# GAIR-Lab/IISAN

Hardware: AMD Instinct MI355X
Metric: items/s (fwd+bwd) ViT-B+BERT-B IISAN uncached, Scientific, bs=128 (higher is better)
Workload: dtype fp16; 1 GPU; Code_Uncached IISAN ViT-base+BERT-base, Amazon-Scientific-shaped synthetic batch, bs=128/GPU (1408 item slots, all encoded), 1xMI355X per rank; global_batch=128, parallelism=dp1, encoder_blocks=all tokens in every block

## Files before the change

### iisan_amd/csrc/common.h

```cpp
#pragma once

#include <hip/hip_runtime.h>
#include <stdint.h>
#include <stdio.h>
#include <string.h>

#include "../../include/iisan_hip.h"

typedef _Float16 h8 __attribute__((ext_vector_type(8)));
typedef _Float16 h4 __attribute__((ext_vector_type(4)));
typedef __bf16 b8 __attribute__((ext_vector_type(8)));
typedef __bf16 b4 __attribute__((ext_vector_type(4)));
typedef float f4 __attribute__((ext_vector_type(4)));
typedef unsigned int u4 __attribute__((ext_vector_type(4)));
typedef unsigned int u2 __attribute__((ext_vector_type(2)));

#define WAVE 64

void iisan_set_error(const char* fmt, ...);

#define IISAN_CHECK_SHAPE(cond, ...)                                                                             \
    do {                                                                                                         \
        if (!(cond)) {                                                                                           \
            iisan_set_error(__VA_ARGS__);                                                                        \
            return IISAN_EBADSHAPE;                                                                              \
        }                                                                                                        \
    } while (0)

#define IISAN_HIP_OK(expr)                                                                                       \
    do {                                                                                                         \
        hipError_t _e = (expr);                                                                                  \
        if (_e != hipSuccess) {                                                                                  \
            iisan_set_error("%s failed at %s:%d: %s", #expr, __FILE__, __LINE__, hipGetErrorString(_e));         \
            return IISAN_EHIP;                                                                                   \
        }                                                                                                        \
    } while (0)

#define IISAN_LAUNCH_OK() IISAN_HIP_OK(hipGetLastError())

struct IisanDevKnob {
    const char* name;
    int64_t def;
    int64_t (*get)();
    void (*set)(int64_t);
};
int iisan_dev_register(const IisanDevKnob& k);
#define IISAN_DEV_KNOB(NAME, VAR)                                                                                \
    static const int iisan_dev_reg_##NAME = iisan_dev_register(IisanDevKnob{                                     \
        #NAME, (int64_t)(VAR), [] { return (int64_t)(VAR); }, [](int64_t v) { VAR = (decltype(VAR))v; }})
#define IISAN_DEV_COUNTER(NAME, VAR)                                                                             \
    static const int iisan_dev_cnt_##NAME = iisan_dev_register(IisanDevKnob{                                     \
        "count:" #NAME, INT64_MIN, [] { return (int64_t)(VAR); }, [](int64_t v) { VAR = (decltype(VAR))v; }})
#define IISAN_DEV_KNOB_FN(NAME, VAR, SET)                                                                        \
    static const int iisan_dev_reg_##NAME = iisan_dev_register(IisanDevKnob{                                     \
        #NAME, (int64_t)(VAR), [] { return (int64_t)(VAR); }, [](int64_t v) { SET; }})

#define IISAN_TRY(expr)                                                                                          \
    do {                                                                                                         \
        int _r = (expr);                                                                                         \
        if (_r != IISAN_OK) return _r;                                                                           \
    } while (0)

constexpr int IISAN_MAX_DEVICES = 64;
int iisan_cu_count();
struct OncePerDevice {
    bool done[IISAN_MAX_DEVICES] = {};
    bool first() {
        int dev = 0;
        if (hipGetDevice(&dev) != hipSuccess || dev < 0 || dev >= IISAN_MAX_DEVICES) return true;
        if (done[dev]) return false;
        done[dev] = true;
        return true;
    }
};

static inline size_t align_up(size_t x, size_t a) { return (x + a - 1) / a * a; }
static inline int64_t ceil_div(int64_t a, int64_t b) { return (a + b - 1) / b; }

struct WsCarver {
    char* base;
    size_t cap, off;
    bool overflow;
    WsCarver(void* p, size_t n) : base((char*)p), cap(n), off(0), overflow(false) {}
    template <typename T>
    T* take(size_t count) {
        size_t bytes = align_up(count * sizeof(T), 256);
        if (base && off + bytes > cap) overflow = true;
        T* r = base ? (T*)(base + off) : nullptr;
        off += bytes;
        return r;
    }
};

struct F16 {
    typedef _Float16 elem;
    typedef h8 v8;
    typedef h4 v4;
    static __device__ __forceinline__ f4 mfma(v8 a, v8 b, f4 c) {
        return __builtin_amdgcn_mfma_f32_16x16x32_f16(a, b, c, 0, 0, 0);
    }
    static __device__ __forceinline__ elem from_f32(float x) { return (_Float16)x; }
    static __device__ __forceinline__ float to_f32(elem x) { return (float)x; }
};
struct BF16 {
    typedef __bf16 elem;
    typedef b8 v8;
    typedef b4 v4;
    static __device__ __forceinline__ f4 mfma(v8 a, v8 b, f4 c) {
        return __builtin_amdgcn_mfma_f32_16x16x32_bf16(a, b, c, 0, 0, 0);
    }
    static __device__ __forceinline__ elem from_f32(float x) { return (__bf16)x; }
    static __device__ __forceinline__ float to_f32(elem x) { return (float)x; }
};

__device__ __forceinline__ float wave_sum(float v) {
#pragma unroll
    for (int o = 32; o > 0; o >>= 1) v += __shfl_xor(v, o, 64);
    return v;
}
__device__ __forceinline__ float wave_max(float v) {
#pragma unroll
    for (int o = 32; o > 0; o >>= 1) v = fmaxf(v, __shfl_xor(v, o, 64));
    return v;
}
__device__ __forceinline__ float gelu_erf(float x) { return 0.5f * x * (1.0f + erff(x * 0.70710678118654752440f)); }
constexpr float GELU_X0 = 5.5f;
__device__ __forceinline__ float gelu_absmin(float x) {
    float r;
    asm("v_min_f32 %0, |%1|, %2" : "=v"(r) : "v"(x), "v"(GELU_X0));
    return r;
}
__device__ __forceinline__ float gelu_relu(float x) {
    float r;
    asm("v_max_f32 %0, 0, %1" : "=v"(r) : "v"(x));
    return r;
}
constexpr float GELU_C0 = 9.170038104e-01f, GELU_C1 = -9.149338305e-02f, GELU_C2 = -3.171720356e-02f, GELU_C3 = -1.111552469e-03f,
                GELU_C4 = 1.940784161e-03f, GELU_C5 = -1.910830324e-04f;
__device__ __forceinline__ float gelu_erf_fast(float x) {
    const float a = gelu_absmin(x);
    float p = fmaf(a, GELU_C5, GELU_C4);
    p = fmaf(p, a, GELU_C3);
    p = fmaf(p, a, GELU_C2);
    p = fmaf(p, a, GELU_C1);
    p = fmaf(p, a, GELU_C0);
    p = p * p; p = p * p; p = p * p;
    return fmaf(-a, p, gelu_relu(x));
}
typedef float f2 __attribute__((ext_vector_type(2)));
template <int NP>
__device__ __forceinline__ void gelu_erf_fast2xN(f2* x) {
    f2 a[NP], p[NP];
#pragma unroll
    for (int k = 0; k < NP; ++k) { a[k][0] = gelu_absmin(x[k][0]); a[k][1] = gelu_absmin(x[k][1]); }
#pragma unroll
    for (int k = 0; k < NP; ++k) p[k] = __builtin_elementwise_fma(a[k], (f2)GELU_C5, (f2)GELU_C4);
#pragma unroll
    for (int k = 0; k < NP; ++k) p[k] = __builtin_elementwise_fma(p[k], a[k], (f2)GELU_C3);
#pragma unroll
    for (int k = 0; k < NP; ++k) p[k] = __builtin_elementwise_fma(p[k], a[k], (f2)GELU_C2);
#pragma unroll
    for (int k = 0; k < NP; ++k) p[k] = __builtin_elementwise_fma(p[k], a[k], (f2)GELU_C1);
#pragma unroll
    for (int k = 0; k < NP; ++k) p[k] = __builtin_elementwise_fma(p[k], a[k], (f2)GELU_C0);
#pragma unroll
    for (int sq = 0; sq < 3; ++sq)
#pragma unroll
        for (int k = 0; k < NP; ++k) p[k] = p[k] * p[k];
#pragma unroll
    for (int k = 0; k < NP; ++k) {
        f2 mx;
        mx[0] = gelu_relu(x[k][0]); mx[1] = gelu_relu(x[k][1]);
        x[k] = __builtin_elementwise_fma(-a[k], p[k], mx);
    }
}
__device__ __forceinline__ void gelu_erf_fast2x8(f2 (&x)[8]) { gelu_erf_fast2xN<8>(x); }
__device__ __forceinline__ float gelu_erf_grad(float x) {
    const float cdf = 0.5f * (1.0f + erff(x * 0.70710678118654752440f));
    const float pdf = 0.39894228040143267794f * __expf(-0.5f * x * x);
    return cdf + x * pdf;
}

__device__ __forceinline__ float drop_scale(uint64_t seed, uint32_t site, uint64_t idx, uint32_t thr24, float inv_keep) {
    uint64_t x = seed + (uint64_t)site * 0x9E3779B97F4A7C15ull + idx * 0xD1B54A32D192ED03ull;
    x ^= x >> 32; x *= 0xD6E8FEB86659FD93ull;
    x ^= x >> 32; x *= 0xD6E8FEB86659FD93ull;
    x ^= x >> 32;
    return ((uint32_t)(x >> 8) & 0xFFFFFFu) >= thr24 ? inv_keep : 0.f;
}
struct DropCfg {
    uint64_t seed;
    uint32_t site, thr24;
    float inv_keep;
};
static inline DropCfg make_drop(uint64_t seed, uint32_t site, float p) {
    DropCfg d;
    d.seed = seed; d.site = site;
    d.thr24 = p > 0.f ? (uint32_t)(p * 16777216.0f) : 0u;
    d.inv_keep = p > 0.f ? 1.0f / (1.0f - p) : 1.0f;
    return d;
}
struct RowKeepNone { static constexpr bool on = false; };
struct RowKeep {
    static constexpr bool on = true;
    DropCfg d;
    int64_t r0;
    int32_t rs;
    __device__ __forceinline__ uint64_t index(int64_t row, int D, int col) const { return (uint64_t)(r0 + row * rs) * (uint64_t)D + (uint64_t)col; }
    __device__ __forceinline__ float operator()(uint64_t idx) const { return drop_scale(d.seed, d.site, idx, d.thr24, d.inv_keep); }
};

__device__ __forceinline__ void glds16(const void* gsrc, void* lds_wave_base) {
    __builtin_amdgcn_global_load_lds((const __attribute__((address_space(1))) void*)gsrc,
                                     (__attribute__((address_space(3))) void*)lds_wave_base, 16, 0, 0);
}

__device__ __forceinline__ int xcd_remap(int bid, int nwg) {
    const int q = nwg >> 3, r = nwg & 7;
    const int xcd = bid & 7, idx = bid >> 3;
    return (xcd < r ? xcd * (q + 1) : r * (q + 1) + (xcd - r) * q) + idx;
}

bool iisan_timing_on(hipStream_t s);
int iisan_timing_class();
void iisan_timing_pre(hipStream_t s, double flops, double bytes);
void iisan_timing_post(hipStream_t s);
inline thread_local int iisan_timing_depth = 0;
struct TimedLaunch {
    hipStream_t s; int cls; bool on;
    TimedLaunch(int cls_, hipStream_t s_, double flops, double bytes)
        : s(s_), cls(cls_), on(cls_ == 1 ? iisan_timing_on(s_) : iisan_timing_class() == 2 && iisan_timing_depth == 0) {
        if (cls == 2) ++iisan_timing_depth;
        if (on) iisan_timing_pre(s, flops, bytes);
    }
    ~TimedLaunch() {
        if (cls == 2) --iisan_timing_depth;
        if (on) iisan_timing_post(s);
    }
};

struct Gemm16Args {
    const void* A;
    const void* W;
    const float* bias;
    void* out;
    const float* resid;
    const float* pos;
    int64_t M;
    int32_t N, K;
    int32_t lda, ldw, ldo;
    int32_t patch_P;
    int32_t qkv_S, qkv_heads;
    int32_t qkv_which0;
    int32_t debug;
    int32_t walk_c, walk_h;
    const float* rowstat;
    float* rowpart;
    const float* inv_a; const float* inv_b;
    int32_t atomic;
    int16_t a_blk32, out_blk32;
    int64_t split_stride;
    const int32_t* skip_last_third;
};
__host__ __device__ static inline int64_t blk32_byte(int64_t m, int64_t c, int64_t C) {
    return ((m >> 5) * (C >> 5) + (c >> 5)) * 2048 + ((c >> 3) & 1) * 1024 + (((c >> 4) & 1) * 32 + (m & 31)) * 16 + (c & 7) * 2;
}
enum { EPI_OUT16 = 0, EPI_GELU16 = 1, EPI_RESID32 = 2, EPI_PATCH32 = 3, EPI_QKVH16 = 4, EPI_F32 = 5, EPI_PATCH16 = 6, EPI_STREAM16 = 7 };
int launch_gemm16(int dtype16, int mode, const Gemm16Args& a, hipStream_t s);
enum { G16_REJECTED = -1, G16_V1 = 0, G16_S256 = 1, G16_H256 = 2 };
int gemm16_route(int dtype16, int mode, const Gemm16Args& a);
bool gemm16_s256_applicable(int mode, const Gemm16Args& a);
int launch_gemm16_s256(int dtype16, int mode, const Gemm16Args& a, hipStream_t s);
bool gemm16_h256_applicable(int mode, const Gemm16Args& a);
int launch_gemm16_h256(int dtype16, int mode, const Gemm16Args& a, hipStream_t s);
int launch_gemm16_f32(const Gemm16Args& a, int ksplit, hipStream_t s);
int launch_layernorm768(int dtype16, const float* x, const float* g, const float* b, float eps, void* out16,
                        float* out32, int64_t rows, int width, hipStream_t s);
int launch_add_layernorm768(int dtype16, const float* x, const void* delta16, const float* g, const float* b, float eps,
                            float* sum32, void* out16, float* out32, int64_t rows, int width, hipStream_t s, const RowKeep* keep = nullptr);
int launch_add2_layernorm768(int dtype16, const float* x, const void* delta16, const void* delta16b, const float* g,
                             const float* b, float eps, float* sum32, void* out16, float* out32, int64_t rows, int width, hipStream_t s,
                             const RowKeep* keep = nullptr);
enum { MX_D1 = 1, MX_D2 = 2, MX_LN = 4, MX_RESV = 8, MX_RESY = 16, MX_SRC32 = 32, MX_CLSONLY = 64, MX_POSROW = 128, MX_STAT = 256, MX_ALIAS = 512, MX_BLK32 = 1024 };
int launch_layernorm768_mixed(int dtype16, int V, const float* x32, void* x16, float* xc, const void* delta16, const void* delta16b,
                              const float* g, const float* b, float eps, void* out16, int64_t items, int Ttok, int width, hipStream_t s,
                              float* stat = nullptr, const RowKeep* keep = nullptr);
struct LnFoldJob { const void* W; const float* bias; const float* g; const float* b; void* Wf; float* bf; int32_t N;
                   int32_t w32;
};
int launch_fold_ln_weights(const LnFoldJob* jobs, int n, hipStream_t s);
int launch_stream_stats_finalize(const float* rowpart, int nslots, int64_t Mpad, void* x16, float* xc, float* rstat, float eps,
                                 int64_t items, int Ttok, hipStream_t s, bool x16_blk32 = false);
int launch_attention16(int dtype16, const void* qkv, const float* key_bias, void* ctx, int64_t items, int S,
                       int heads, hipStream_t s);
bool attention16_dma_routed(const float* key_bias, int S);
int launch_attention16_dma(int dtype16, const void* qkv, void* ctx, int64_t items, int S, int heads, hipStream_t s);
int launch_attention_cls16(int dtype16, const void* qkv, const float* key_bias, void* ctx_cls, int64_t items, int S,
                           int heads, hipStream_t s, const void* q_cls = nullptr);
int launch_vit_im2col(int dtype16, const void* img, int img_u8, void* out, int64_t M, int C, int R, int p, hipStream_t s);
int launch_vit_im2col_indexed(int dtype16, const uint8_t* catalogue, int64_t rows, const int64_t* index, void* out, int64_t M, int C,
                              int R, int p, hipStream_t s);
int launch_vit_cls_rows(float* X, const float* cls, const float* pos, int64_t M, int T, int D, hipStream_t s);
int launch_bert_embed_ln(int dtype16, const int64_t* text, const float* word, const float* pos, const float* type0,
                         const float* g, const float* b, float eps, float* X, void* H, float* key_bias, int64_t M,
                         int W, int vocab, int width, hipStream_t s, void* X16 = nullptr, float* Xc = nullptr, const RowKeep* keep = nullptr);
int launch_bert_embed_ln_indexed(int dtype16, const int64_t* table, int64_t rows, const int64_t* index, const float* word, const float* pos,
                                 const float* type0, const float* g, const float* b, float eps, float* X, void* H, float* key_bias,
                                 int64_t M, int W, int vocab, int width, hipStream_t s, void* X16 = nullptr, float* Xc = nullptr,
                                 const RowKeep* keep = nullptr);
int launch_attention16_drop(int dtype16, const void* qkv, const float* key_bias, void* ctx, int64_t items, int S, int heads,
                            const DropCfg& drop, int64_t slot0, bool cls_only, const void* q_cls, hipStream_t s);
void iisan_count_bert_drop();
int launch_gather_cls(const float* X, float* taps, int64_t M, int T, int D, int n_taps, int k, hipStream_t s);
int launch_gather_rows16(const void* H, void* out, int64_t M, int T, int D, hipStream_t s);

struct Gemm32Prob;
size_t gemm_x3_ws_bytes(int64_t M, int64_t N, int64_t K);
bool gemm_x3_applicable(const Gemm32Prob& p, int flags);
int launch_gemm_x3(const Gemm32Prob& p, int flags, void* ws, size_t ws_bytes, hipStream_t s);
size_t gemm_x3_group_ws_bytes(const int64_t* M, const int64_t* N, const int64_t* K, int n);
int launch_gemm_x3_group(const Gemm32Prob* probs, int n, int flags, void* ws, size_t ws_bytes, hipStream_t s);
int gemm_x3_group_max();
double gemm_x3_get_min_flops();
void gemm_x3_set_min_flops(double f);

struct X3pArgs {
    const _Float16* A2; const _Float16* B2;
    int64_t M; int32_t N, kp;
    const float* bias; const float* resid; float* out; int32_t ldo;
    const float* inv_a; const float* inv_b;
    const int32_t* lo_a; const int32_t* lo_b;
    int64_t split_stride;
};
int launch_gemm16_x3p(const X3pArgs& a, int ksplit, hipStream_t s);
int x3p_tile_n(int64_t M, int64_t N);

struct AmaxBatch { const float* x[16]; int64_t rows[16], cols[16], ld[16]; uint32_t* out[16]; };
int launch_amax_batch(const AmaxBatch& b, int n, hipStream_t s);

struct FuseOperands {
    const float* a; const float* b; const float* prev;
    int64_t lda, ldb, ldp;
    const float* gate;
    int32_t D, type;
};
struct Gemm32Prob {
    const float* A; const float* B; const float* bias; const float* resid; const float* act_src; float* C;
    int64_t M; int32_t N; int64_t K;
    int32_t lda, ldb, ldc, ldr;
    DropCfg drop;
    int64_t ksplit_stride;
    uint32_t* amax_a; uint32_t* amax_b;
    int32_t amax_a_ready, amax_b_ready;
    int32_t exact16_a, exact16_b;
    uint32_t* x3_zeroed;
    float* colsum_a;
};
struct N64FDesc {
    FuseOperands f;
    float* F;
    const float* W; int32_t ldw;
    const float* bias;
    float* U; float* A;
    int64_t M; int32_t K;
};
bool gemm32_n64f_ok(const N64FDesc* d, int n);
int launch_gemm32_n64f(const N64FDesc* d, int n, int gelu, hipStream_t s);
struct K64Gate { const float* gate; const float* ga; const float* go; int64_t ldga, ldgo; float* dgate; int32_t scale_prev, store; float* d2; int64_t ldd2; int32_t d2_is_b; };
bool gemm32_k64_gate_ok(const Gemm32Prob* probs, const K64Gate* gates, int nprob);
int launch_gemm32_k64_gate(const Gemm32Prob* probs, const K64Gate* gates, int nprob, hipStream_t s);
void gemm32_set_scratch(float* ws, size_t floats);
enum {
    G32_TA = 1,
    G32_TB = 2,
    G32_RELU = 4,
    G32_GELU = 8,
    G32_ACCUM = 16,
    G32_MUL_RELU_MASK = 32,
    G32_MUL_GELU_GRAD = 64,
    G32_PREACT = 128,
    G32_HINT_B_EXACT16 = 1024,
    G32_DROPOUT = 256,
};
int launch_gemm32(const Gemm32Prob* probs, int nprob, int flags, hipStream_t s);
int launch_colsum(const float* const* X, float* const* out, const int64_t* M, const int32_t* N, const int32_t* ld,
                  int nprob, hipStream_t s);

struct SanbTowerDesc {
    FuseOperands f;
    const float* Wd; const float* bd; const float* Wu; const float* bu;
    float* F; float* U; float* A; float* O;
    const float* dO; const float* Upre; float* dU; float* dprev; float* da; float* db; float* dgate; float* dbu; float* dbd;
};
bool sanb_fused_ok(int D, int down);
int launch_sanb_fwd(const SanbTowerDesc* towers, int n, int64_t M, int gelu, hipStream_t s);
int launch_sanb_bwd(const SanbTowerDesc* towers, int n, int64_t M, int gelu, hipStream_t s);
int launch_sanb_transpose(const float* const* in, float* const* out, const int32_t* rows, const int32_t* cols, int n, hipStream_t s);

struct SasFusedPtrs {
    float* Z0; float* X0;
    float* Q[8]; float* K[8]; float* V[8]; float* P[8]; float* C[8]; float* Zattn[8]; float* X1[8]; float* Hf[8]; float* Zffn[8]; float* X2[8];
};
bool sasrec_fused_ok(const iisan_sasrec_cfg* cfg);
bool sasrec_fused_shape_ok(const iisan_sasrec_cfg* cfg);
int launch_sasrec_fused_fwd(const iisan_sasrec_cfg* cfg, const float* x, const float* log_mask, int64_t B, const void* const* params,
                            float* y, const SasFusedPtrs& w, hipStream_t s);
int64_t sasrec_fused_slab_floats(const iisan_sasrec_cfg* cfg, int64_t B);
int launch_sasrec_fused_bwd(const iisan_sasrec_cfg* cfg, const float* log_mask, int64_t B, const void* const* params, const float* dy,
                            float* dx, void* const* grads, const SasFusedPtrs& w, float* slab, hipStream_t s);
```

### iisan_amd/csrc/gemm32.hip

```cpp
#include "common.h"

namespace {

constexpr int TN = 64, TK = 64, LD = 66;
__host__ __device__ constexpr int ldt(int rows) { return rows == 16 ? 48 : rows + 16; }
__host__ __device__ constexpr int smem_floats(int rows) { return rows * LD > TK * ldt(rows) ? rows * LD : TK * ldt(rows); }
typedef float f2v __attribute__((ext_vector_type(2)));

constexpr int G32_MAXP = 6;
struct Gemm32Batch {
    Gemm32Prob p[G32_MAXP];
};

template <int ROWS>
__device__ __forceinline__ void load_tile(f4 (&v)[ROWS / 16], const float* __restrict__ src, int ld, bool trans, int64_t row0,
                                          int64_t rows, int64_t k0, int64_t kend, int tid) {
    constexpr int TPR = ROWS / 4;
#pragma unroll
    for (int i = 0; i < ROWS / 16; ++i) {
        v[i] = (f4){0.f, 0.f, 0.f, 0.f};
        if (!trans) {
            const int64_t row = row0 + (tid >> 4) + 16 * i, k = k0 + (tid & 15) * 4;
            if (row < rows && k < kend) {
                const float* p = src + row * ld + k;
                if (k + 3 < kend && (((uintptr_t)p) & 15) == 0) {
                    v[i] = *(const f4*)p;
                } else {
#pragma unroll
                    for (int e = 0; e < 4; ++e)
                        if (k + e < kend) v[i][e] = p[e];
                }
            }
        } else {
            const int64_t k = k0 + tid / TPR + (256 / TPR) * i, row = row0 + (tid % TPR) * 4;
            if (k < kend && row < rows) {
                const float* p = src + k * ld + row;
                if (row + 3 < rows && (((uintptr_t)p) & 15) == 0) {
                    v[i] = *(const f4*)p;
                } else {
#pragma unroll
                    for (int e = 0; e < 4; ++e)
                        if (row + e < rows) v[i][e] = p[e];
                }
            }
        }
    }
}
template <int ROWS>
__device__ __forceinline__ void store_tile(float* S, const f4 (&v)[ROWS / 16], bool trans, int tid) {
    constexpr int TPR = ROWS / 4;
#pragma unroll
    for (int i = 0; i < ROWS / 16; ++i) {
        if (!trans) {
            float* d = S + ((tid >> 4) + 16 * i) * LD + (tid & 15) * 4;
            *(f2v*)d = (f2v){v[i][0], v[i][1]};
            *(f2v*)(d + 2) = (f2v){v[i][2], v[i][3]};
        } else {
            *(f4*)(S + (tid / TPR + (256 / TPR) * i) * ldt(ROWS) + (tid % TPR) * 4) = v[i];
        }
    }
}

template <int FLAGS, int TMV, bool FAST, int DEPTHV = 2>
__global__ __launch_bounds__(256) void gemm32_kernel(Gemm32Batch batch, int epi) {
    constexpr int TM = TMV;
    constexpr int WM = TMV >= 32 ? 2 : 1, WN = 4 / WM, FM = TMV / 16 / WM, FN = 4 / WN;
    __shared__ __attribute__((aligned(16))) float As_[smem_floats(TM)];
    __shared__ __attribute__((aligned(16))) float Bs_[smem_floats(TN)];
    float (*As)[LD] = (float (*)[LD])As_;
    const Gemm32Prob& p = batch.p[blockIdx.z];
    const int tiles_n = (p.N + TN - 1) / TN;
    const int64_t tiles_m = (p.M + TM - 1) / TM;
    if ((int64_t)blockIdx.x >= tiles_m * tiles_n) return;
    const int64_t tile_m = blockIdx.x / tiles_n;
    const int tile_n = blockIdx.x - tile_m * tiles_n;
    const int64_t m0 = tile_m * TM;
    const int n0 = tile_n * TN;

    const int64_t ktiles = (p.K + TK - 1) / TK;
    const int64_t per = (ktiles + gridDim.y - 1) / gridDim.y;
    const int64_t kbeg = (int64_t)blockIdx.y * per * TK;
    int64_t kend = kbeg + per * TK;
    if (kend > p.K) kend = p.K;
    if (kbeg >= kend && blockIdx.y > 0) return;

    const int tid = threadIdx.x, lane = tid & 63, wave = tid >> 6;
    const int wm = wave / WN, wn = wave % WN;
    const int fi = lane & 15, fk = lane >> 4;
    constexpr bool TA = (FLAGS & G32_TA) != 0, TB = (FLAGS & G32_TB) != 0;

    constexpr int KA = (FM * FN >= 4) ? 1 : 4 / (FM * FN);
    f4 acc[KA][FM][FN];
#pragma unroll
    for (int q = 0; q < KA; ++q)
#pragma unroll
        for (int a = 0; a < FM; ++a)
#pragma unroll
            for (int b = 0; b < FN; ++b) acc[q][a][b] = (f4){0.f, 0.f, 0.f, 0.f};

    constexpr int DEPTH = DEPTHV;
    f4 ra[DEPTH][TM / 16], rb[DEPTH][4];
    constexpr int TPRA = TM / 4, TPRB = TN / 4;
    const float* pa = TA ? p.A + (kbeg + tid / TPRA) * p.lda + m0 + (tid % TPRA) * 4 : p.A + (m0 + (tid >> 4)) * p.lda + kbeg + (tid & 15) * 4;
    const float* pb = TB ? p.B + (kbeg + tid / TPRB) * p.ldb + n0 + (tid % TPRB) * 4 : p.B + (int64_t)(n0 + (tid >> 4)) * p.ldb + kbeg + (tid & 15) * 4;
    const int64_t sia = TA ? (int64_t)(256 / TPRA) * p.lda : (int64_t)16 * p.lda, sib = TB ? (int64_t)(256 / TPRB) * p.ldb : (int64_t)16 * p.ldb;
    const int64_t ska = TA ? (int64_t)TK * p.lda : TK, skb = TB ? (int64_t)TK * p.ldb : TK;
    const int64_t last_t = (kend - kbeg - 1) / TK;
    auto fetch = [&](int slot, int64_t k) {
        if constexpr (FAST) {
            int64_t t = (k - kbeg) / TK;
            t = t < last_t ? t : last_t;
#pragma unroll
            for (int i = 0; i < TM / 16; ++i) ra[slot][i] = *(const f4*)(pa + t * ska + i * sia);
#pragma unroll
            for (int i = 0; i < 4; ++i) rb[slot][i] = *(const f4*)(pb + t * skb + i * sib);
            return;
        }
        if (k < kend) {
            if constexpr (FAST) {
            } else {
                load_tile<TM>(ra[slot], p.A, p.lda, TA, m0, p.M, k, kend, tid);
                load_tile<TN>(rb[slot], p.B, p.ldb, TB, n0, p.N, k, kend, tid);
            }
        }
    };
    constexpr int NP = TM / 16 + 4;
    const float* const pa_u = TA ? p.A + kbeg * p.lda + m0 : p.A + m0 * p.lda + kbeg;
    const float* const pb_u = TB ? p.B + kbeg * p.ldb + n0 : p.B + (int64_t)n0 * p.ldb + kbeg;
    uint32_t voa[TM / 16], vob[4];
#pragma unroll
    for (int i = 0; i < TM / 16; ++i)
        voa[i] = (uint32_t)(((TA ? (int64_t)(tid / TPRA) * p.lda + (tid % TPRA) * 4 : (int64_t)(tid >> 4) * p.lda + (tid & 15) * 4) + i * sia) * 4);
#pragma unroll
    for (int i = 0; i < 4; ++i)
        vob[i] = (uint32_t)(((TB ? (int64_t)(tid / TPRB) * p.ldb + (tid % TPRB) * 4 : (int64_t)(tid >> 4) * p.ldb + (tid & 15) * 4) + i * sib) * 4);
    auto fetch_piece = [&](int slot, int64_t k, int i) {
        int64_t t = (k - kbeg) / TK;
        t = t < last_t ? t : last_t;
        if (i < TM / 16) ra[slot][i] = *(const f4*)((const char*)(pa_u + t * ska) + voa[i]);
        else rb[slot][i - TM / 16] = *(const f4*)((const char*)(pb_u + t * skb) + vob[i - TM / 16]);
    };
#pragma unroll
    for (int u = 0; u < DEPTH; ++u) fetch(u, kbeg + (int64_t)u * TK);
    for (int64_t kb = kbeg; kb < kend; kb += (int64_t)DEPTH * TK) {
#pragma unroll
        for (int u = 0; u < DEPTH; ++u) {
            const int64_t k0 = kb + (int64_t)u * TK;
            if (k0 < kend) {
                store_tile<TM>(As_, ra[u], TA, tid);
                store_tile<TN>(Bs_, rb[u], TB, tid);
                __syncthreads();
                if constexpr (!FAST) fetch(u, k0 + (int64_t)DEPTH * TK);
                const int ksteps = (kend - k0 >= TK) ? TK / 4 : (int)((kend - k0 + 3) / 4);
                auto kstep = [&](int ks0) {
#pragma unroll
                    for (int q = 0; q < KA; ++q) {
                        const int ks = ks0 + q;
                        float a[FM], b[FN];
#pragma unroll
                        for (int f = 0; f < FM; ++f)
                            a[f] = TA ? As_[(ks * 4 + fk) * ldt(TM) + wm * 16 * FM + f * 16 + fi] : As_[(wm * 16 * FM + f * 16 + fi) * LD + ks * 4 + fk];
#pragma unroll
                        for (int f = 0; f < FN; ++f)
                            b[f] = TB ? Bs_[(ks * 4 + fk) * ldt(TN) + wn * 16 * FN + f * 16 + fi] : Bs_[(wn * 16 * FN + f * 16 + fi) * LD + ks * 4 + fk];
#pragma unroll
                        for (int mf = 0; mf < FM; ++mf)
#pragma unroll
                            for (int nf = 0; nf < FN; ++nf)
                                acc[q][mf][nf] = __builtin_amdgcn_mfma_f32_16x16x4f32(a[mf], b[nf], acc[q][mf][nf], 0, 0, 0);
                    }
                };
                if (FAST || ksteps == TK / 4) {
                    float ac[FM], bc[FN];
                    auto frag = [&](int ks, float (&a)[FM], float (&b)[FN]) {
#pragma unroll
                        for (int f = 0; f < FM; ++f)
                            a[f] = TA ? As_[(ks * 4 + fk) * ldt(TM) + wm * 16 * FM + f * 16 + fi] : As_[(wm * 16 * FM + f * 16 + fi) * LD + ks * 4 + fk];
#pragma unroll
                        for (int f = 0; f < FN; ++f)
                            b[f] = TB ? Bs_[(ks * 4 + fk) * ldt(TN) + wn * 16 * FN + f * 16 + fi] : Bs_[(wn * 16 * FN + f * 16 + fi) * LD + ks * 4 + fk];
                    };
                    frag(0, ac, bc);
#pragma unroll
                    for (int ks = 0; ks < TK / 4; ++ks) {
                        float an[FM], bn[FN];
                        frag(ks + 1 < TK / 4 ? ks + 1 : ks, an, bn);
                        __builtin_amdgcn_sched_barrier(0);
#pragma unroll
                        for (int mf = 0; mf < FM; ++mf)
#pragma unroll
                            for (int nf = 0; nf < FN; ++nf)
                                acc[ks % KA][mf][nf] = __builtin_amdgcn_mfma_f32_16x16x4f32(ac[mf], bc[nf], acc[ks % KA][mf][nf], 0, 0, 0);
                        if constexpr (FAST) {
                            if ((ks & 1) && (ks >> 1) < NP) fetch_piece(u, k0 + (int64_t)DEPTH * TK, ks >> 1);
                        }
                        __builtin_amdgcn_sched_barrier(0);
#pragma unroll
                        for (int f = 0; f < FM; ++f) ac[f] = an[f];
#pragma unroll
                        for (int f = 0; f < FN; ++f) bc[f] = bn[f];
                    }
                } else {
                    for (int ks0 = 0; ks0 < ksteps; ks0 += KA) kstep(ks0);
                }
                __syncthreads();
            }
        }
    }

    const bool first_split = blockIdx.y == 0;
    float* const Cp = p.C + (int64_t)blockIdx.y * p.ksplit_stride;
    constexpr bool ACC = (FLAGS & G32_ACCUM) != 0;
    const bool vec_ok = !ACC && n0 + TN <= p.N && (p.ldc & 3) == 0 && ((uintptr_t)p.C & 15) == 0 &&
                        (!p.resid || ((p.ldr & 3) == 0 && ((uintptr_t)p.resid & 15) == 0)) &&
                        (!p.act_src || ((uintptr_t)p.act_src & 15) == 0) && (!p.bias || ((uintptr_t)p.bias & 15) == 0);
    if (vec_ok) {
#pragma unroll
        for (int mf = 0; mf < FM; ++mf)
#pragma unroll
            for (int nf = 0; nf < FN; ++nf)
#pragma unroll
                for (int r = 0; r < 4; ++r) {
                    float v = acc[0][mf][nf][r];
#pragma unroll
                    for (int q = 1; q < KA; ++q) v += acc[q][mf][nf][r];
                    As[wm * 16 * FM + mf * 16 + fk * 4 + r][wn * 16 * FN + nf * 16 + fi] = v;
                }
        __syncthreads();
        for (int idx = tid; idx < TM * 16; idx += 256) {
            const int row = idx >> 4, c4 = (idx & 15) * 4;
            const int64_t m = m0 + row;
            if (m >= p.M) continue;
            const int n = n0 + c4;
            const f2v lo = *(const f2v*)&As[row][c4], hi = *(const f2v*)&As[row][c4 + 2];
            f4 v = {lo[0], lo[1], hi[0], hi[1]};
            if (p.bias && first_split) v += *(const f4*)(p.bias + n);
            const int64_t ci = m * p.ldc + n;
            if (epi & G32_PREACT) *(f4*)((float*)p.act_src + ci) = v;
            f4 act = {0.f, 0.f, 0.f, 0.f};
            if (epi & (G32_MUL_RELU_MASK | G32_MUL_GELU_GRAD)) act = *(const f4*)(p.act_src + ci);
#pragma unroll
            for (int e = 0; e < 4; ++e) {
                float x = v[e];
                if (epi & G32_RELU) x = fmaxf(x, 0.f);
                if (epi & G32_GELU) x = gelu_erf(x);
                if (epi & G32_MUL_RELU_MASK) x = act[e] > 0.f ? x : 0.f;
                if (epi & G32_MUL_GELU_GRAD) x *= gelu_erf_grad(act[e]);
                if (epi & G32_DROPOUT) x *= drop_scale(p.drop.seed, p.drop.site, (uint64_t)(ci + e), p.drop.thr24, p.drop.inv_keep);
                v[e] = x;
            }
            if (p.resid && first_split) v += *(const f4*)(p.resid + m * p.ldr + n);
            *(f4*)(Cp + ci) = v;
        }
        return;
    }
#pragma unroll
    for (int mf = 0; mf < FM; ++mf)
#pragma unroll
        for (int nf = 0; nf < FN; ++nf) {
            const int n = n0 + wn * 16 * FN + nf * 16 + fi;
            if (n >= p.N) continue;
            const float bias = (p.bias && first_split) ? p.bias[n] : 0.f;
#pragma unroll
            for (int r = 0; r < 4; ++r) {
                const int64_t m = m0 + wm * 16 * FM + mf * 16 + fk * 4 + r;
                if (m >= p.M) continue;
                float v = acc[0][mf][nf][r];
#pragma unroll
                for (int q = 1; q < KA; ++q) v += acc[q][mf][nf][r];
                v += bias;
                if (epi & G32_PREACT) ((float*)p.act_src)[m * p.ldc + n] = v;
                if (epi & G32_RELU) v = fmaxf(v, 0.f);
                if (epi & G32_GELU) v = gelu_erf(v);
                if (epi & G32_MUL_RELU_MASK) v = p.act_src[m * p.ldc + n] > 0.f ? v : 0.f;
                if (epi & G32_MUL_GELU_GRAD) v *= gelu_erf_grad(p.act_src[m * p.ldc + n]);
                if (epi & G32_DROPOUT) v *= drop_scale(p.drop.seed, p.drop.site, (uint64_t)(m * p.ldc + n), p.drop.thr24, p.drop.inv_keep);
                if (p.resid && first_split) v += p.resid[m * p.ldr + n];
                if constexpr (ACC)
                    atomicAdd(p.C + m * p.ldc + n, v);
                else
                    Cp[m * p.ldc + n] = v;
            }
        }
}

__global__ __launch_bounds__(256, 2) void gemm32_dw_kernel(Gemm32Batch batch) {
    __shared__ __attribute__((aligned(16))) float sm[2][2][64 * 64];
    const Gemm32Prob& p = batch.p[blockIdx.z];
    const int tiles_n = p.N >> 6;
    const int64_t tiles_m = p.M >> 6;
    if ((int64_t)blockIdx.x >= tiles_m * tiles_n) return;
    const int64_t tile_m = blockIdx.x / tiles_n;
    const int tile_n = (int)(blockIdx.x - tile_m * tiles_n);
    const int64_t m0 = tile_m * 64;
    const int n0 = tile_n * 64;
    const int64_t ktiles = p.K / TK;
    const int64_t per = (ktiles + gridDim.y - 1) / gridDim.y;
    const int64_t kt0 = (int64_t)blockIdx.y * per;
    int64_t kt1 = kt0 + per;
    if (kt1 > ktiles) kt1 = ktiles;
    if (kt0 >= kt1) return;
    const int tid = threadIdx.x, lane = tid & 63;
    const int wave = __builtin_amdgcn_readfirstlane(tid >> 6);
    const int i16 = lane & 15, kq = lane >> 4;
    const float* const a_u = p.A + kt0 * TK * p.lda + m0;
    const float* const b_u = p.B + kt0 * TK * p.ldb + n0;
    uint32_t voa[4], vob[4];
#pragma unroll
    for (int q = 0; q < 4; ++q) {
        voa[q] = (uint32_t)((((int64_t)(tid >> 4) + 16 * q) * p.lda + (tid & 15) * 4) * 4);
        vob[q] = (uint32_t)((((int64_t)(tid >> 4) + 16 * q) * p.ldb + (tid & 15) * 4) * 4);
    }
    const int64_t nt = kt1 - kt0;
    f4 st[2][8];
    auto piece = [&](int slot, int64_t t, int q) {
        t = t < nt ? t : nt - 1;
        if (q < 4) st[slot][q] = *(const f4*)((const char*)(a_u + t * TK * p.lda) + voa[q]);
        else st[slot][q] = *(const f4*)((const char*)(b_u + t * TK * p.ldb) + vob[q - 4]);
    };
#pragma unroll
    for (int q = 0; q < 8; ++q) piece(0, 0, q);
#pragma unroll
    for (int q = 0; q < 8; ++q) piece(1, 1, q);
    f4 acc[4][4];
#pragma unroll
    for (int e = 0; e < 4; ++e)
#pragma unroll
        for (int f = 0; f < 4; ++f) acc[e][f] = (f4){0.f, 0.f, 0.f, 0.f};
    const int sw = (tid >> 4) * 64 + (tid & 15) * 4;
    const int rd = (16 * wave + kq) * 64 + 4 * i16;
    const bool do_cs = p.colsum_a != nullptr && tile_n == 0;
    f4 csum = {0.f, 0.f, 0.f, 0.f};
    auto tile = [&](int64_t t, int slot) {
        float* bufA = sm[t & 1][0];
        float* bufB = sm[t & 1][1];
#pragma unroll
        for (int q = 0; q < 4; ++q) {
            *(f4*)(bufA + sw + 16 * 64 * q) = st[slot][q];
            *(f4*)(bufB + sw + 16 * 64 * q) = st[slot][4 + q];
            if (do_cs) csum += st[slot][q];
        }
        __builtin_amdgcn_sched_barrier(0);
        __syncthreads();
        __builtin_amdgcn_sched_barrier(0);
        f4 a = *(const f4*)(bufA + rd), b = *(const f4*)(bufB + rd);
#pragma unroll
        for (int s = 0; s < 4; ++s) {
            const f4 an = *(const f4*)(bufA + rd + 4 * 64 * (s < 3 ? s + 1 : s)), bn = *(const f4*)(bufB + rd + 4 * 64 * (s < 3 ? s + 1 : s));
            __builtin_amdgcn_sched_barrier(0);
#pragma unroll
            for (int e = 0; e < 4; ++e) {
#pragma unroll
                for (int f = 0; f < 4; ++f) acc[e][f] = __builtin_amdgcn_mfma_f32_16x16x4f32(a[e], b[f], acc[e][f], 0, 0, 0);
                if (e & 1) {
                    __builtin_amdgcn_sched_barrier(0);
                    piece(slot, t + 2, 2 * s + (e >> 1));
                    __builtin_amdgcn_sched_barrier(0);
                }
            }
            __builtin_amdgcn_sched_barrier(0);
            a = an; b = bn;
        }
    };
    int64_t t = 0;
#pragma unroll 1
    for (; t + 2 <= nt; t += 2) { tile(t, 0); tile(t + 1, 1); }
    if (t < nt) tile(t, 0);
    __syncthreads();
    float* red = &sm[0][0][0] + wave * 4096;
#pragma unroll
    for (int e = 0; e < 4; ++e)
#pragma unroll
        for (int r = 0; r < 4; ++r)
            *(f4*)(red + (16 * kq + 4 * r + e) * 64 + 4 * i16) = (f4){acc[e][0][r], acc[e][1][r], acc[e][2][r], acc[e][3][r]};
    __syncthreads();
    float* const Cp = p.C + (int64_t)blockIdx.y * p.ksplit_stride;
    const float* all = &sm[0][0][0];
#pragma unroll
    for (int q = 0; q < 4; ++q) {
        const int id = tid + 256 * q;
        const int o = (id >> 4) * 64 + (id & 15) * 4;
        const f4 v = (*(const f4*)(all + o) + *(const f4*)(all + 4096 + o)) + (*(const f4*)(all + 8192 + o) + *(const f4*)(all + 12288 + o));
        *(f4*)(Cp + (m0 + (id >> 4)) * p.ldc + n0 + (id & 15) * 4) = v;
    }
    if (do_cs) {
        __syncthreads();
        float* cs = &sm[0][0][0];
        *(f4*)(cs + (tid >> 4) * 64 + (tid & 15) * 4) = csum;
        __syncthreads();
        if (tid < 64) {
            float v = 0.f;
#pragma unroll
            for (int r = 0; r < 16; ++r) v += cs[r * 64 + tid];
            Cp[p.M * p.N + m0 + tid] = v;
        }
    }
}

struct N64FProb {
    const float* a; const float* b; const float* prev; int64_t lda, ldb, ldp; const float* gate; int32_t type;
    float* F; const float* W; int32_t ldw; const float* bias; float* U; float* A; float* P; int64_t pstride; int64_t M; int32_t K;
};
struct N64FBatch { N64FProb p[3]; int32_t gelu; int32_t rpw; };

__global__ __launch_bounds__(256, 2) void gemm32_n64f_kernel(N64FBatch batch) {
    __shared__ __attribute__((aligned(16))) float wl[2][64 * 68];
    const N64FProb& p = batch.p[blockIdx.z];
    const int64_t m0 = (int64_t)blockIdx.x * batch.rpw;
    if (m0 >= p.M) return;
    const int ktiles = p.K >> 6;
    const int per = (ktiles + (int)gridDim.y - 1) / (int)gridDim.y;
    const int kt0 = (int)blockIdx.y * per;
    int kt1 = kt0 + per;
    if (kt1 > ktiles) kt1 = ktiles;
    if (kt0 >= kt1) return;
    const int nt = kt1 - kt0;
    const int tid = threadIdx.x, lane = tid & 63;
    const int wave = __builtin_amdgcn_readfirstlane(tid >> 6);
    const int j = lane & 15, g = lane >> 4;
    const int64_t mj = m0 + 16 * wave + j;
    const int64_t mrow = mj < p.M ? mj : p.M - 1;
    const bool live = mj < p.M && 16 * wave + j < batch.rpw;
    const bool wave_on = 16 * wave < batch.rpw;
    const bool gated = p.gate != nullptr;
    const float gv = gated ? 1.0f / (1.0f + __expf(-p.gate[0] / 0.1f)) : 1.0f;
    const float ca = gated ? gv : 1.f, cb = gated ? 1.f - gv : 1.f;
    const bool has_b = p.type == 1;
    const float cp = p.prev ? (p.type == 0 ? cb : 1.f) : 0.f;
    const float* arow = p.a + mrow * p.lda + 4 * g;
    const float* prow = p.prev ? p.prev + mrow * p.ldp + 4 * g : arow;
    const float* brow = has_b ? p.b + mrow * p.ldb + 4 * g : arow;
    float* frow = p.F + mrow * (int64_t)p.K + 4 * g;
    const float* wsrc = p.W + (int64_t)(tid >> 4) * p.ldw + (tid & 15) * 4;
    const int64_t wq = (int64_t)16 * p.ldw;
    const int sw = (tid >> 4) * 68 + (tid & 15) * 4;
    f4 wst[4], an[4], pn[4], bn[4];
    auto piece = [&](int t, int q) {
        const int kk = (kt0 + (t < nt ? t : nt - 1)) * 64;
        const int s = q & 3;
        if (q < 4) an[s] = *(const f4*)(arow + kk + 16 * s);
        else if (q < 8) pn[s] = *(const f4*)(prow + kk + 16 * s);
        else if (q < 12) { if (has_b) bn[s] = *(const f4*)(brow + kk + 16 * s); }
        else wst[s] = *(const f4*)(wsrc + kk + s * wq);
    };
#pragma unroll
    for (int q = 0; q < 16; ++q) piece(0, q);
    f4 acc[4];
#pragma unroll
    for (int q = 0; q < 4; ++q) acc[q] = (f4){0.f, 0.f, 0.f, 0.f};
    const int lw = j * 68 + 4 * g;
#pragma unroll 1
    for (int t = 0; t < nt; ++t) {
        float* buf = wl[t & 1];
        const int kk = (kt0 + t) * 64;
        f4 xa[4];
#pragma unroll
        for (int s = 0; s < 4; ++s) {
            *(f4*)(buf + sw + 16 * 68 * s) = wst[s];
            f4 f = cp * pn[s] + ca * an[s];
            if (has_b) f += cb * bn[s];
            xa[s] = f;
            if (live) *(f4*)(frow + kk + 16 * s) = f;
        }
        __builtin_amdgcn_sched_barrier(0);
        __syncthreads();
        __builtin_amdgcn_sched_barrier(0);
        const float* wb = buf + lw;
        if (wave_on) {
#pragma unroll
            for (int s = 0; s < 4; ++s) {
                f4 w[4];
#pragma unroll
                for (int f = 0; f < 4; ++f) w[f] = *(const f4*)(wb + 16 * f * 68 + 16 * s);
#pragma unroll
                for (int e = 0; e < 4; ++e) {
#pragma unroll
                    for (int f = 0; f < 4; ++f) acc[f] = __builtin_amdgcn_mfma_f32_16x16x4f32(w[f][e], xa[s][e], acc[f], 0, 0, 0);
                    __builtin_amdgcn_sched_barrier(0);
                    piece(t + 1, 4 * s + e);
                    __builtin_amdgcn_sched_barrier(0);
                }
            }
        } else {
#pragma unroll
            for (int q = 12; q < 16; ++q) piece(t + 1, q);
        }
    }
    if (!live) return;
    if (gridDim.y > 1) {
        float* pr = p.P + (int64_t)blockIdx.y * p.pstride + mrow * 64 + 4 * g;
#pragma unroll
        for (int f = 0; f < 4; ++f) *(f4*)(pr + 16 * f) = acc[f];
        return;
    }
#pragma unroll
    for (int f = 0; f < 4; ++f) {
        const int n = 16 * f + 4 * g;
        f4 v = acc[f] + *(const f4*)(p.bias + n);
        *(f4*)(p.U + mrow * 64 + n) = v;
#pragma unroll
        for (int e = 0; e < 4; ++e) v[e] = batch.gelu ? gelu_erf(v[e]) : fmaxf(v[e], 0.f);
        *(f4*)(p.A + mrow * 64 + n) = v;
    }
}

struct K64Prob {
    const float* A; const float* W; const float* bias; const float* resid; float* C; int64_t M; int32_t N, lda, ldw, ldc, ldr;
    const float* gate; const float* ga; const float* go; int64_t ldga, ldgo; float* dgate; int32_t scale_prev, store;
    float* d2; int64_t ldd2; int32_t d2_is_b;
};
struct K64Batch { K64Prob p[4]; };

template <bool TBV, bool GATE = false>
__global__ __launch_bounds__(256, 2) void gemm32_k64_kernel(K64Batch batch, int nblk) {
    extern __shared__ __attribute__((aligned(16))) float wlds[];
    __shared__ float gred[4];
    const K64Prob& p = batch.p[blockIdx.z];
    const int c0 = (int)blockIdx.y * nblk * 64;
    if ((int64_t)blockIdx.x * 64 >= p.M || c0 >= p.N) return;
    int nb = (p.N - c0) >> 6;
    nb = nb < nblk ? nb : nblk;
    const int cols = nb * 64;
    const int tid = threadIdx.x, lane = tid & 63;
    const int wave = __builtin_amdgcn_readfirstlane(tid >> 6);
    const int j = lane & 15, g = lane >> 4;
    const int stride = TBV ? cols + 4 : 68;
    {
        const int per_row = TBV ? cols / 4 : 16;
        const int pieces = 16 * cols;
        f4 t[16];
#pragma unroll
        for (int q = 0; q < 16; ++q) {
            int id = tid + 256 * q;
            id = id < pieces ? id : pieces - 1;
            const int r = id / per_row, c = id - r * per_row;
            t[q] = TBV ? *(const f4*)(p.W + (int64_t)r * p.ldw + c0 + 4 * c) : *(const f4*)(p.W + (int64_t)(c0 + r) * p.ldw + 4 * c);
        }
#pragma unroll
        for (int q = 0; q < 16; ++q) {
            const int id = tid + 256 * q;
            if (id < pieces) {
                const int r = id / per_row, c = id - r * per_row;
                *(f4*)(wlds + r * stride + 4 * c) = t[q];
            }
        }
    }
    const bool has_r = p.resid != nullptr, has_b = p.bias != nullptr;
    float gpart = 0.f, gval = 0.f;
    if constexpr (GATE) gval = 1.0f / (1.0f + __expf(-p.gate[0] / 0.1f));
    const float cdp = (GATE && p.scale_prev) ? 1.f - gval : 1.f;
    const float cgo = (GATE && p.go) ? 1.f : 0.f;
    const float cd2 = GATE ? (p.d2_is_b ? 1.f - gval : gval) : 0.f;
    const float* wl = wlds + (TBV ? (16 * g) * stride + 4 * (4 * (j & 3) + (j >> 2)) : j * stride + 4 * g);
    __syncthreads();
#pragma unroll 1
    for (int64_t m0 = (int64_t)blockIdx.x * 64; m0 < p.M; m0 += (int64_t)gridDim.x * 64) {
    const int64_t mj = m0 + 16 * wave + j;
    const int64_t mrow = mj < p.M ? mj : p.M - 1;
    const bool live = mj < p.M;
    f4 xa[4];
    {
        const float* ar = p.A + mrow * p.lda + (TBV ? 16 * g : 4 * g);
#pragma unroll
        for (int q = 0; q < 4; ++q) xa[q] = *(const f4*)(ar + (TBV ? 4 * q : 16 * q));
    }
    const int ocol = c0 + 4 * g;
    float* crow = p.C + mrow * p.ldc + ocol;
    const float* rrow = has_r ? p.resid + mrow * p.ldr + ocol : crow;
    const float* brow = has_b ? p.bias + ocol : p.W + 4 * g;
    const float* garow = GATE ? p.ga + mrow * p.ldga + ocol : nullptr;
    const float* gorow = GATE ? (p.go ? p.go + mrow * p.ldgo + ocol : p.ga + mrow * p.ldga + ocol) : nullptr;
    f4 rn[4];
#pragma unroll
    for (int q = 0; q < 4; ++q) rn[q] = *(const f4*)(rrow + 16 * q);
#pragma unroll 1
    for (int t = 0; t < nb; ++t) {
        f4 wc[16];
        {
            const float* wb = wl + (TBV ? 64 * t : 64 * t * stride);
#pragma unroll
            for (int q1 = 0; q1 < (TBV ? 16 : 4); ++q1)
#pragma unroll
                for (int q2 = 0; q2 < (TBV ? 1 : 4); ++q2)
                    wc[TBV ? q1 : 4 * q1 + q2] = *(const f4*)(wb + q1 * (TBV ? stride : 16 * stride) + 16 * q2);
        }
        f4 rv[4], bv[4];
        const int tn = t + 1 < nb ? t + 1 : t;
#pragma unroll
        for (int q = 0; q < 4; ++q) {
            rv[q] = rn[q];
            bv[q] = *(const f4*)(brow + 64 * t + 16 * q);
        }
#pragma unroll
        for (int q = 0; q < 4; ++q) rn[q] = *(const f4*)(rrow + 64 * tn + 16 * q);
        f4 gav[4], gov[4];
        if constexpr (GATE) {
#pragma unroll
            for (int q = 0; q < 4; ++q) {
                gav[q] = *(const f4*)(garow + 64 * t + 16 * q);
                gov[q] = *(const f4*)(gorow + 64 * t + 16 * q);
            }
        }
        __builtin_amdgcn_sched_barrier(0);
        f4 acc[4];
#pragma unroll
        for (int q = 0; q < 4; ++q) acc[q] = (f4){0.f, 0.f, 0.f, 0.f};
        if constexpr (TBV) {
#pragma unroll
            for (int s = 0; s < 16; ++s)
#pragma unroll
                for (int e = 0; e < 4; ++e) acc[e] = __builtin_amdgcn_mfma_f32_16x16x4f32(wc[s][e], xa[s >> 2][s & 3], acc[e], 0, 0, 0);
        } else {
#pragma unroll
            for (int s = 0; s < 4; ++s)
#pragma unroll
                for (int e = 0; e < 4; ++e)
#pragma unroll
                    for (int f = 0; f < 4; ++f) acc[f] = __builtin_amdgcn_mfma_f32_16x16x4f32(wc[4 * f + s][e], xa[s][e], acc[f], 0, 0, 0);
        }
        __builtin_amdgcn_sched_barrier(0);
#pragma unroll
        for (int q = 0; q < 4; ++q) {
            const f4 v = TBV ? (f4){acc[0][q], acc[1][q], acc[2][q], acc[3][q]} : acc[q];
            const f4 z = {0.f, 0.f, 0.f, 0.f};
            const f4 o = v + ((has_b ? bv[q] : z) + (has_r ? rv[q] : z));
            if constexpr (GATE) {
                if (live) {
                    const f4 d = gav[q] - cgo * gov[q];
                    gpart += (o[0] * d[0] + o[1] * d[1]) + (o[2] * d[2] + o[3] * d[3]);
                    if (p.store) *(f4*)(crow + 64 * t + 16 * q) = o * cdp;
                    if (p.d2) *(f4*)(p.d2 + mrow * p.ldd2 + ocol + 64 * t + 16 * q) = o * cd2;
                }
            } else {
                if (live) *(f4*)(crow + 64 * t + 16 * q) = o;
            }
        }
    }
    }
    if constexpr (GATE) {
        gpart = wave_sum(gpart);
        if (lane == 0) gred[wave] = gpart;
        __syncthreads();
        if (tid == 0) atomicAdd(p.dgate, ((gred[0] + gred[1]) + (gred[2] + gred[3])) * gval * (1.f - gval) / 0.1f);
    }
}

struct ColsumBatch {
    const float* X[4];
    float* out[4];
    int64_t M[4];
    int32_t N[4], ld[4];
};
__global__ __launch_bounds__(256) void colsum_kernel(ColsumBatch b, int rows_per_block) {
    __shared__ float part[4][64];
    const int z = blockIdx.z;
    const int c = threadIdx.x & 63, rl = threadIdx.x >> 6;
    const int n = blockIdx.x * 64 + c;
    const int64_t r0 = (int64_t)blockIdx.y * rows_per_block;
    int64_t r1 = r0 + rows_per_block;
    if (r1 > b.M[z]) r1 = b.M[z];
    float s = 0.f;
    if (n < b.N[z]) {
        const float* xp = b.X[z] + n;
        const int64_t ld = b.ld[z];
        float part8[8] = {0.f, 0.f, 0.f, 0.f, 0.f, 0.f, 0.f, 0.f};
        int64_t r = r0 + rl;
        for (; r + 28 < r1; r += 32) {
#pragma unroll
            for (int u = 0; u < 8; ++u) part8[u] += xp[(r + 4 * u) * ld];
        }
        for (; r < r1; r += 4) s += xp[r * ld];
        s += ((part8[0] + part8[1]) + (part8[2] + part8[3])) + ((part8[4] + part8[5]) + (part8[6] + part8[7]));
    }
    part[rl][c] = s;
    __syncthreads();
    if (rl == 0 && n < b.N[z] && r0 < b.M[z]) atomicAdd(b.out[z] + n, part[0][c] + part[1][c] + part[2][c] + part[3][c]);
}

struct ReduceBatch { Gemm32Prob p[G32_MAXP]; const float* P[G32_MAXP]; int64_t stride[G32_MAXP]; int32_t ns[G32_MAXP]; float* cs[G32_MAXP]; };
__global__ __launch_bounds__(256) void gemm32_reduce_kernel(ReduceBatch rb, int ks_launch, int epi) {
    const Gemm32Prob& p = rb.p[blockIdx.z];
    const int ks = ks_launch < rb.ns[blockIdx.z] ? ks_launch : rb.ns[blockIdx.z];
    const float* P = rb.P[blockIdx.z];
    const int64_t stride = rb.stride[blockIdx.z], total = p.M * p.N;
    if (rb.cs[blockIdx.z]) {
        for (int64_t m = (int64_t)blockIdx.x * blockDim.x + threadIdx.x; m < p.M; m += (int64_t)gridDim.x * blockDim.x) {
            float v = 0.f;
            for (int y = 0; y < ks; ++y) v += P[(int64_t)y * stride + total + m];
            rb.cs[blockIdx.z][m] += v;
        }
    }
    if (epi == 0 && !p.bias && (p.N & 3) == 0 && (p.ldc & 3) == 0 && (!p.resid || (p.ldr & 3) == 0)) {
        const int64_t total4 = total / 4;
        const int n4 = p.N / 4;
        for (int64_t i = (int64_t)blockIdx.x * blockDim.x + threadIdx.x; i < total4; i += (int64_t)gridDim.x * blockDim.x) {
            const int64_t m = i / n4;
            const int n = (int)(i - m * n4) * 4;
            f4 acc[8];
#pragma unroll
            for (int u = 0; u < 8; ++u) acc[u] = (f4){0.f, 0.f, 0.f, 0.f};
            int y = 0;
            for (; y + 8 <= ks; y += 8) {
#pragma unroll
                for (int u = 0; u < 8; ++u) acc[u] += *(const f4*)(P + (int64_t)(y + u) * stride + 4 * i);
            }
            for (int u = 0; y < ks; ++y, ++u) acc[u] += *(const f4*)(P + (int64_t)y * stride + 4 * i);
            f4 v = ((acc[0] + acc[1]) + (acc[2] + acc[3])) + ((acc[4] + acc[5]) + (acc[6] + acc[7]));
            if (p.resid) v += *(const f4*)(p.resid + m * p.ldr + n);
            *(f4*)(p.C + m * p.ldc + n) = v;
        }
        return;
    }
    for (int64_t i = (int64_t)blockIdx.x * blockDim.x + threadIdx.x; i < total; i += (int64_t)gridDim.x * blockDim.x) {
        const int64_t m = i / p.N;
        const int n = (int)(i - m * p.N);
        float v = P[i];
        for (int y = 1; y < ks; ++y) v += P[y * stride + i];
        if (p.bias) v += p.bias[n];
        const int64_t ci = m * p.ldc + n;
        if (epi & G32_PREACT) ((float*)p.act_src)[ci] = v;
        if (epi & G32_RELU) v = fmaxf(v, 0.f);
        if (epi & G32_GELU) v = gelu_erf(v);
        if (epi & G32_MUL_RELU_MASK) v = p.act_src[ci] > 0.f ? v : 0.f;
        if (epi & G32_MUL_GELU_GRAD) v *= gelu_erf_grad(p.act_src[ci]);
        if (epi & G32_DROPOUT) v *= drop_scale(p.drop.seed, p.drop.site, (uint64_t)ci, p.drop.thr24, p.drop.inv_keep);
        if (p.resid) v += p.resid[m * p.ldr + n];
        p.C[ci] = v;
    }
}

thread_local float* g_scratch = nullptr;
thread_local size_t g_scratch_floats = 0;

template <int FLAGS, bool FAST, int DEPTH>
void launch_tiled(const Gemm32Batch& b, dim3 grid, int tm, int epi, hipStream_t s) {
    if (tm == 64) hipLaunchKernelGGL((gemm32_kernel<FLAGS, 64, FAST, DEPTH>), grid, dim3(256), 0, s, b, epi);
    else if (tm == 32) hipLaunchKernelGGL((gemm32_kernel<FLAGS, 32, FAST, DEPTH>), grid, dim3(256), 0, s, b, epi);
    else hipLaunchKernelGGL((gemm32_kernel<FLAGS, 16, FAST, DEPTH>), grid, dim3(256), 0, s, b, epi);
}
template <int FLAGS>
int launch_flags(const Gemm32Batch& b, dim3 grid, int tm, int epi, bool fast, bool deep, hipStream_t s) {
    constexpr bool DW = (FLAGS & (G32_TA | G32_TB)) == (G32_TA | G32_TB);
    if (DW && deep) launch_tiled<FLAGS, true, DW ? 3 : 2>(b, grid, tm, epi, s);
    else if (fast) launch_tiled<FLAGS, true, 2>(b, grid, tm, epi, s);
    else launch_tiled<FLAGS, false, 2>(b, grid, tm, epi, s);
    IISAN_LAUNCH_OK();
    return IISAN_OK;
}
constexpr int (*g_tiled[8])(const Gemm32Batch&, dim3, int, int, bool, bool, hipStream_t) = {
    launch_flags<0>, launch_flags<G32_TA>, launch_flags<G32_TB>, launch_flags<G32_TA | G32_TB>,
    launch_flags<G32_ACCUM>, launch_flags<G32_TA | G32_ACCUM>, launch_flags<G32_TB | G32_ACCUM>, launch_flags<G32_TA | G32_TB | G32_ACCUM>};

int nonempty_splits(int64_t ktiles, int splits) { return (int)ceil_div(ktiles, ceil_div(ktiles, (int64_t)splits)); }

int launch_reduce(ReduceBatch& rb, int n, int splitk, int epi, hipStream_t s) {
    int64_t max_mn = 0;
    for (int i = 0; i < n; ++i) {
        rb.ns[i] = nonempty_splits(ceil_div(rb.p[i].K, (int64_t)TK), splitk);
        if (rb.p[i].M * rb.p[i].N > max_mn) max_mn = rb.p[i].M * rb.p[i].N;
    }
    int64_t blocks = ceil_div(max_mn, 256);
    if (blocks > 2048) blocks = 2048;
    hipLaunchKernelGGL(gemm32_reduce_kernel, dim3((unsigned)blocks, 1, (unsigned)n), dim3(256), 0, s, rb, splitk, epi);
    IISAN_LAUNCH_OK();
    return IISAN_OK;
}

}

static int g_use_k64 = 1, g_use_dw = 1;
static int64_t g_cnt_n64f = 0, g_cnt_k64 = 0, g_cnt_dw = 0;
IISAN_DEV_COUNTER(gemm32_n64f, g_cnt_n64f);
IISAN_DEV_COUNTER(gemm32_k64, g_cnt_k64);
IISAN_DEV_COUNTER(gemm32_dw, g_cnt_dw);
IISAN_DEV_KNOB(gemm32_dw, g_use_dw);
static int g_dw_splits = 0;
IISAN_DEV_KNOB(gemm32_dw_splits, g_dw_splits);
IISAN_DEV_KNOB(gemm32_k64, g_use_k64);

void gemm32_set_scratch(float* ws, size_t floats) { g_scratch = ws; g_scratch_floats = floats; }

static int g_use_n64f = 1;
IISAN_DEV_KNOB(gemm32_n64f, g_use_n64f);
bool gemm32_n64f_ok(const N64FDesc* d, int n) {
    if (!g_use_n64f || n < 1 || n > 3) return false;
    for (int i = 0; i < n; ++i) {
        const N64FDesc& q = d[i];
        const FuseOperands& f = q.f;
        if (q.K < 256 || (q.K & 63) || (f.lda & 3) || (q.ldw & 3) || (f.prev && (f.ldp & 3)) || (f.type == 1 && (!f.b || (f.ldb & 3))) || !f.a || !q.bias ||
            (((uintptr_t)f.a | (uintptr_t)f.b | (uintptr_t)f.prev | (uintptr_t)q.F | (uintptr_t)q.W | (uintptr_t)q.bias | (uintptr_t)q.U | (uintptr_t)q.A) & 15))
            return false;
    }
    return true;
}
static void fill(N64FProb& q, const N64FDesc& d) {
    q.a = d.f.a; q.b = d.f.b; q.prev = d.f.prev; q.lda = d.f.lda; q.ldb = d.f.ldb; q.ldp = d.f.ldp; q.gate = d.f.gate; q.type = d.f.type;
    q.F = d.F; q.W = d.W; q.ldw = d.ldw; q.bias = d.bias; q.U = d.U; q.A = d.A; q.M = d.M; q.K = d.K;
}
static int launch_gemm32_n64f_impl(const N64FDesc* d, int n, int gelu, hipStream_t s) {
    IISAN_CHECK_SHAPE(gemm32_n64f_ok(d, n), "gemm32_n64f: unsupported problem");
    N64FBatch nb{};
    nb.gelu = gelu;
    int64_t maxM = 0;
    int max_k = 0;
    for (int i = 0; i < n; ++i) {
        fill(nb.p[i], d[i]);
        if (d[i].M > maxM) maxM = d[i].M;
        if (d[i].K > max_k) max_k = d[i].K;
    }
    const int cus = iisan_cu_count();
    int rpw = 64;
    if (g_use_n64f != 2 && maxM % cus == 0 && maxM / cus > 32 && maxM / cus < 64) rpw = (int)(maxM / cus);
    nb.rpw = rpw;
    const int64_t rt = ceil_div(maxM, rpw);
    IISAN_CHECK_SHAPE(rt < (1ll << 31), "gemm32: grid too large");
    int ks = 1;
    if (g_scratch && rt * n < 384) {
        ks = max_k / (4 * TK);
        if (ks > 16) ks = 16;
        while (ks >= 2) {
            int64_t need = 0;
            for (int i = 0; i < n; ++i) need += (int64_t)ks * (int64_t)align_up((size_t)(d[i].M * 64), 64);
            if ((size_t)need <= g_scratch_floats) break;
            ks >>= 1;
        }
        if (ks < 2) ks = 1;
    }
    if (ks >= 2) {
        int64_t off = 0;
        for (int i = 0; i < n; ++i) {
            nb.p[i].P = g_scratch + off;
            nb.p[i].pstride = (int64_t)align_up((size_t)(d[i].M * 64), 64);
            off += ks * nb.p[i].pstride;
        }
    }
    ++g_cnt_n64f;
    hipLaunchKernelGGL(gemm32_n64f_kernel, dim3((unsigned)rt, (unsigned)ks, (unsigned)n), dim3(256), 0, s, nb);
    IISAN_LAUNCH_OK();
    if (ks < 2) return IISAN_OK;
    ReduceBatch rb{};
    for (int i = 0; i < n; ++i) {
        Gemm32Prob& q = rb.p[i];
        q.C = d[i].A; q.ldc = 64; q.bias = d[i].bias; q.act_src = d[i].U; q.M = d[i].M; q.N = 64; q.K = d[i].K; q.ldr = 64;
        rb.P[i] = nb.p[i].P;
        rb.stride[i] = nb.p[i].pstride;
    }
    return launch_reduce(rb, n, ks, (gelu ? G32_GELU : G32_RELU) | G32_PREACT, s);
}

static bool k64_shape_ok(const Gemm32Prob& q) {
    return q.K == 64 && q.N >= 256 && (q.N & 63) == 0 && !q.act_src && q.ksplit_stride == 0 &&
           (q.lda & 3) == 0 && (q.ldb & 3) == 0 && (q.ldc & 3) == 0 && (!q.resid || (q.ldr & 3) == 0) &&
           (((uintptr_t)q.A | (uintptr_t)q.B | (uintptr_t)q.C | (uintptr_t)q.resid | (uintptr_t)q.bias) & 15) == 0;
}
struct K64Grid { int64_t rt; int nblk, ny; };
static K64Grid k64_grid(const Gemm32Prob* probs, int nprob) {
    int64_t maxM = 0;
    int maxnb = 0;
    for (int i = 0; i < nprob; ++i) {
        if (probs[i].M > maxM) maxM = probs[i].M;
        if ((probs[i].N >> 6) > maxnb) maxnb = probs[i].N >> 6;
    }
    K64Grid g;
    g.rt = ceil_div(maxM, 64);
    g.nblk = 4;
    while (g.nblk > 1 && g.rt * ceil_div(maxnb, g.nblk) * nprob < 1024) g.nblk >>= 1;
    g.ny = (int)ceil_div(maxnb, g.nblk);
    return g;
}
static void fill_k64(K64Batch& kb, const Gemm32Prob* probs, int nprob) {
    for (int i = 0; i < nprob; ++i) {
        const Gemm32Prob& q = probs[i];
        K64Prob& k = kb.p[i];
        k = K64Prob{};
        k.A = q.A; k.W = q.B; k.bias = q.bias; k.resid = q.resid; k.C = q.C; k.M = q.M; k.N = q.N;
        k.lda = q.lda; k.ldw = q.ldb; k.ldc = q.ldc; k.ldr = q.ldr;
    }
}
static int g_use_k64_gate = 1;
IISAN_DEV_KNOB(gemm32_k64_gate, g_use_k64_gate);
bool gemm32_k64_gate_ok(const Gemm32Prob* probs, const K64Gate* gates, int nprob) {
    if (!g_use_k64 || !g_use_k64_gate || nprob < 1 || nprob > 4) return false;
    for (int i = 0; i < nprob; ++i) {
        const K64Gate& g = gates[i];
        if (!k64_shape_ok(probs[i]) || !probs[i].resid || !g.gate || !g.ga || !g.dgate || (g.ldga & 3) || (g.go && (g.ldgo & 3)) || (g.d2 && ((g.ldd2 & 3) || ((uintptr_t)g.d2 & 15))) ||
            (((uintptr_t)g.ga | (uintptr_t)g.go) & 15))
            return false;
    }
    return true;
}
static int launch_gemm32_k64_gate_impl(const Gemm32Prob* probs, const K64Gate* gates, int nprob, hipStream_t s) {
    IISAN_CHECK_SHAPE(gemm32_k64_gate_ok(probs, gates, nprob), "gemm32_k64_gate: unsupported problem");
    K64Batch kb{};
    fill_k64(kb, probs, nprob);
    for (int i = 0; i < nprob; ++i) {
        K64Prob& k = kb.p[i];
        k.gate = gates[i].gate; k.ga = gates[i].ga; k.go = gates[i].go; k.ldga = gates[i].ldga; k.ldgo = gates[i].ldgo;
        k.dgate = gates[i].dgate; k.scale_prev = gates[i].scale_prev; k.store = gates[i].store;
        k.d2 = gates[i].d2; k.ldd2 = gates[i].ldd2; k.d2_is_b = gates[i].d2_is_b;
    }
    const K64Grid g = k64_grid(probs, nprob);
    IISAN_CHECK_SHAPE(g.rt < (1ll << 31), "gemm32: grid too large");
    const dim3 grid((unsigned)g.rt, (unsigned)g.ny, (unsigned)nprob);
    const size_t lds = (size_t)64 * (64 * g.nblk + 4) * sizeof(float);
    static OncePerDevice attr;
    if (attr.first())
        IISAN_HIP_OK(hipFuncSetAttribute((const void*)gemm32_k64_kernel<true, true>, hipFuncAttributeMaxDynamicSharedMemorySize, 4 * 64 * 68 * 4));
    ++g_cnt_k64;
    hipLaunchKernelGGL((gemm32_k64_kernel<true, true>), grid, dim3(256), lds, s, kb, g.nblk);
    IISAN_LAUNCH_OK();
    return IISAN_OK;
}

enum { G32K_REJECTED = -1, G32K_TILED = 0, G32K_K64 = 1, G32K_DW = 2,
       G32K_SPLIT_K64 = 3 };
enum { G32S_NONE = 0,
       G32S_EPILOGUE = 1,
       G32S_ADD_C = 2 };
enum { G32C_NONE = 0, G32C_FOLDED = 1, G32C_OWN_LAUNCH = 2 };
struct Gemm32Plan {
    int kernel;
    int tm, splitk;
    int scratch;
    bool fast, deep;
    int colsum;
    int nblk;
    int64_t gx; int gy, gz;
    int nk64;
};

static constexpr int g_tm_thresh = 512, g_splitk_target = 1024;

static int64_t partial_floats(const Gemm32Prob& q, bool with_colsum) {
    return (int64_t)align_up((size_t)(q.M * q.N + (with_colsum && q.colsum_a ? q.M : 0)), 64);
}
static bool partials_fit(const Gemm32Prob* probs, int nprob, int splitk, bool with_colsum, size_t scratch_floats) {
    int64_t need = 0;
    for (int i = 0; i < nprob; ++i) need += (int64_t)splitk * partial_floats(probs[i], with_colsum);
    return (size_t)need <= scratch_floats;
}

static Gemm32Plan plan_gemm32(const Gemm32Prob* probs, int nprob, int flags, size_t scratch_floats) {
    Gemm32Plan pl{};
    pl.kernel = G32K_REJECTED;
    if (nprob < 1 || nprob > G32_MAXP) { iisan_set_error("gemm32: 1..%d problems per launch (got %d)", G32_MAXP, nprob); return pl; }
    int64_t min_k = INT64_MAX, max_k = 0;
    bool any_colsum = false;
    for (int i = 0; i < nprob; ++i) {
        if (!(probs[i].M > 0 && probs[i].N > 0 && probs[i].K > 0)) { iisan_set_error("gemm32: empty problem %d", i); return pl; }
        if (probs[i].K < min_k) min_k = probs[i].K;
        if (probs[i].K > max_k) max_k = probs[i].K;
        any_colsum = any_colsum || probs[i].colsum_a;
    }
    const bool have_scratch = scratch_floats > 0;
    if ((flags & ~G32_TB) == 0 && g_use_k64) {
        int nk64 = 0;
        for (int i = 0; i < nprob; ++i) nk64 += k64_shape_ok(probs[i]) ? 1 : 0;
        if (nk64 > 0 && nk64 < nprob) { pl.kernel = G32K_SPLIT_K64; pl.nk64 = nk64; return pl; }
        if (nk64 == nprob && nprob <= 4) {
            const K64Grid g = k64_grid(probs, nprob);
            if (g.rt >= (1ll << 31)) { iisan_set_error("gemm32: grid too large"); return pl; }
            pl.kernel = G32K_K64; pl.nblk = g.nblk; pl.gx = g.rt; pl.gy = g.ny; pl.gz = nprob;
            return pl;
        }
    }
    auto tiles_for = [&](int tm) {
        int64_t mt = 0;
        for (int i = 0; i < nprob; ++i) {
            const int64_t t = ceil_div(probs[i].M, tm) * ceil_div(probs[i].N, TN);
            if (t > mt) mt = t;
        }
        return mt;
    };
    pl.tm = 64;
    if (!(flags & G32_ACCUM) && tiles_for(64) * nprob < g_tm_thresh) pl.tm = tiles_for(32) * nprob >= g_tm_thresh ? 32 : 16;
    const int64_t max_tiles = tiles_for(pl.tm);
    if (max_tiles >= (1ll << 31)) { iisan_set_error("gemm32: grid too large"); return pl; }
    pl.gx = max_tiles; pl.gz = nprob;
    bool dw_ok = g_use_dw && flags == (G32_TA | G32_TB | G32_ACCUM) && have_scratch;
    for (int i = 0; i < nprob && dw_ok; ++i) {
        const Gemm32Prob& q = probs[i];
        dw_ok = (q.M & 63) == 0 && (q.N & 63) == 0 && (q.K & 63) == 0 && q.K >= 4 * TK && (q.lda & 3) == 0 && (q.ldb & 3) == 0 &&
                (((uintptr_t)q.A | (uintptr_t)q.B) & 15) == 0;
    }
    pl.splitk = 1;
    if (flags & G32_ACCUM) {
        int64_t want = ceil_div(g_splitk_target, max_tiles * nprob);
        if (dw_ok) {
            int64_t sum_tiles = 0;
            for (int i = 0; i < nprob; ++i) sum_tiles += (probs[i].M >> 6) * (probs[i].N >> 6);
            const int cus = iisan_cu_count();
            want = ((int64_t)cus + sum_tiles / 2) / sum_tiles;
            if (nprob > 3) want = ((int64_t)2 * cus + sum_tiles / 2) / sum_tiles;
            if (g_dw_splits > 0 && nprob > 3) want = g_dw_splits;
        }
        const int64_t maxs = ceil_div(min_k, 2 * TK);
        pl.splitk = (int)(want < 1 ? 1 : (want > maxs ? maxs : want));
        if (have_scratch && (pl.splitk >= 2 || dw_ok)) {
            pl.splitk = nonempty_splits(ceil_div(min_k, (int64_t)TK), pl.splitk);
            if (partials_fit(probs, nprob, pl.splitk, dw_ok, scratch_floats)) pl.scratch = G32S_ADD_C;
        }
    } else if (have_scratch && max_tiles <= 192) {
        int ks = (int)(max_k / (8 * TK));
        if (ks > 8) ks = 8;
        if (ks >= 2 && partials_fit(probs, nprob, ks, false, scratch_floats)) { pl.splitk = ks; pl.scratch = G32S_EPILOGUE; }
    }
    pl.gy = pl.splitk;
    if (dw_ok && pl.scratch == G32S_ADD_C) {
        pl.kernel = G32K_DW;
        pl.colsum = any_colsum ? G32C_FOLDED : G32C_NONE;
        return pl;
    }
    pl.kernel = G32K_TILED;
    pl.fast = true;
    for (int i = 0; i < nprob && pl.fast; ++i) {
        const Gemm32Prob& q = probs[i];
        pl.fast = q.M % pl.tm == 0 && q.N % TN == 0 && q.K % TK == 0 &&
                  (q.lda & 3) == 0 && (q.ldb & 3) == 0 && ((uintptr_t)q.A & 15) == 0 && ((uintptr_t)q.B & 15) == 0;
    }
    pl.deep = pl.fast && (flags & (G32_TA | G32_TB)) == (G32_TA | G32_TB) && min_k >= 4096;
    pl.colsum = (any_colsum && (flags & G32_TA)) ? G32C_OWN_LAUNCH : G32C_NONE;
    return pl;
}

static int launch_gemm32_impl(const Gemm32Prob* probs, int nprob, int flags, hipStream_t s) {
    const Gemm32Plan pl = plan_gemm32(probs, nprob, flags, g_scratch ? g_scratch_floats : 0);
    if (pl.kernel == G32K_REJECTED) return IISAN_EBADSHAPE;
    if (pl.kernel == G32K_SPLIT_K64) {
        Gemm32Prob yes[G32_MAXP], no[G32_MAXP];
        int ny = 0, nn = 0;
        for (int i = 0; i < nprob; ++i) { if (k64_shape_ok(probs[i])) yes[ny++] = probs[i]; else no[nn++] = probs[i]; }
        IISAN_TRY(launch_gemm32_impl(yes, ny, flags, s));
        return launch_gemm32_impl(no, nn, flags, s);
    }
    const dim3 grid((unsigned)pl.gx, (unsigned)pl.gy, (unsigned)pl.gz);
    if (pl.kernel == G32K_K64) {
        K64Batch kb{};
        fill_k64(kb, probs, nprob);
        const size_t lds = (size_t)64 * pl.nblk * 68 * sizeof(float);
        static OncePerDevice attr;
        if (attr.first()) {
            IISAN_HIP_OK(hipFuncSetAttribute((const void*)gemm32_k64_kernel<true>, hipFuncAttributeMaxDynamicSharedMemorySize, 4 * 64 * 68 * 4));
            IISAN_HIP_OK(hipFuncSetAttribute((const void*)gemm32_k64_kernel<false>, hipFuncAttributeMaxDynamicSharedMemorySize, 4 * 64 * 68 * 4));
        }
        ++g_cnt_k64;
        if (flags & G32_TB) hipLaunchKernelGGL(gemm32_k64_kernel<true>, grid, dim3(256), lds, s, kb, pl.nblk);
        else hipLaunchKernelGGL(gemm32_k64_kernel<false>, grid, dim3(256), lds, s, kb, pl.nblk);
        IISAN_LAUNCH_OK();
        return IISAN_OK;
    }
    Gemm32Batch b{};
    for (int i = 0; i < nprob; ++i) b.p[i] = probs[i];
    if (pl.scratch != G32S_NONE) {
        int64_t off = 0;
        for (int i = 0; i < nprob; ++i) {
            Gemm32Prob& q = b.p[i];
            q.C = g_scratch + off; q.ldc = q.N; q.bias = nullptr; q.resid = nullptr; q.act_src = nullptr;
            q.ksplit_stride = partial_floats(q, pl.kernel == G32K_DW);
            off += pl.splitk * q.ksplit_stride;
        }
    }
    const int epi = flags & ~(G32_TA | G32_TB | G32_ACCUM);
    if (pl.kernel == G32K_DW) {
        ++g_cnt_dw;
        hipLaunchKernelGGL(gemm32_dw_kernel, grid, dim3(256), 0, s, b);
        IISAN_LAUNCH_OK();
    } else {
        const int structural = flags & (G32_TA | G32_TB | (pl.scratch == G32S_NONE ? G32_ACCUM : 0));
        const int kepi = pl.scratch == G32S_NONE ? epi : 0;
        IISAN_TRY(g_tiled[(structural & 3) | (structural & G32_ACCUM ? 4 : 0)](b, grid, pl.tm, kepi, pl.fast, pl.deep, s));
    }
    if (pl.colsum == G32C_OWN_LAUNCH) {
        const float* X[G32_MAXP]; float* O[G32_MAXP]; int64_t Ms[G32_MAXP]; int32_t Ns[G32_MAXP], lds[G32_MAXP];
        int n = 0;
        for (int i = 0; i < nprob; ++i)
            if (probs[i].colsum_a) { X[n] = probs[i].A; O[n] = probs[i].colsum_a; Ms[n] = probs[i].K; Ns[n] = (int32_t)probs[i].M; lds[n] = probs[i].lda; ++n; }
        for (int i = 0; i < n; i += 4) IISAN_TRY(launch_colsum(X + i, O + i, Ms + i, Ns + i, lds + i, n - i < 4 ? n - i : 4, s));
    }
    if (pl.scratch == G32S_NONE) return IISAN_OK;
    ReduceBatch rb{};
    for (int i = 0; i < nprob; ++i) {
        rb.p[i] = probs[i];
        if (pl.scratch == G32S_ADD_C) {
            rb.p[i].resid = probs[i].C; rb.p[i].ldr = probs[i].ldc; rb.p[i].bias = nullptr;
        }
        rb.P[i] = b.p[i].C;
        rb.stride[i] = b.p[i].ksplit_stride;
        rb.cs[i] = pl.colsum == G32C_FOLDED ? probs[i].colsum_a : nullptr;
    }
    return launch_reduce(rb, nprob, pl.splitk, epi, s);
}

extern "C" int32_t iisan_gemm32_plan(const int64_t* M, const int32_t* N, const int64_t* K, int32_t nprob, int32_t flags, int64_t scratch_floats,
                                     int32_t with_colsum, int32_t* plan12) {
    static float present[4];
    Gemm32Prob p[G32_MAXP] = {};
    for (int i = 0; i < nprob && i < G32_MAXP; ++i) {
        p[i].M = M[i]; p[i].N = N[i]; p[i].K = K[i];
        p[i].lda = (int32_t)((flags & G32_TA) ? M[i] : K[i]);
        p[i].ldb = (int32_t)((flags & G32_TB) ? N[i] : K[i]);
        p[i].ldc = N[i]; p[i].ldr = N[i];
        if (flags & (G32_PREACT | G32_MUL_RELU_MASK | G32_MUL_GELU_GRAD)) p[i].act_src = present;
        if (with_colsum) p[i].colsum_a = present;
    }
    const Gemm32Plan pl = plan_gemm32(p, nprob, flags, scratch_floats > 0 ? (size_t)scratch_floats : 0);
    const int64_t v[12] = {pl.kernel, pl.tm, pl.splitk, pl.scratch, pl.fast, pl.deep, pl.colsum, pl.nblk, pl.gx, pl.gy, pl.gz, pl.nk64};
    for (int i = 0; i < 12; ++i) plan12[i] = (int32_t)v[i];
    return pl.kernel;
}

int launch_gemm32(const Gemm32Prob* probs, int nprob, int flags, hipStream_t s) {
    double fl = 0, by = 0;
    for (int i = 0; i < nprob && i < G32_MAXP; ++i) {
        fl += 2.0 * (double)probs[i].M * probs[i].N * (double)probs[i].K;
        by += 4.0 * ((double)probs[i].M * probs[i].K + (double)probs[i].N * probs[i].K + (double)probs[i].M * probs[i].N);
    }
    TimedLaunch t(2, s, fl, by);
    return launch_gemm32_impl(probs, nprob, flags, s);
}
int launch_gemm32_n64f(const N64FDesc* d, int n, int gelu, hipStream_t s) {
    double fl = 0, by = 0;
    for (int i = 0; i < n; ++i) {
        fl += 2.0 * (double)d[i].M * 64.0 * d[i].K;
        by += 4.0 * ((double)d[i].M * d[i].K * ((d[i].f.a ? 1 : 0) + (d[i].f.b ? 1 : 0) + (d[i].f.prev ? 1 : 0) + 1) + 64.0 * d[i].K + 2.0 * d[i].M * 64.0);
    }
    TimedLaunch t(2, s, fl, by);
    return launch_gemm32_n64f_impl(d, n, gelu, s);
}
int launch_gemm32_k64_gate(const Gemm32Prob* probs, const K64Gate* gates, int nprob, hipStream_t s) {
    double fl = 0, by = 0;
    for (int i = 0; i < nprob; ++i) {
        fl += 2.0 * (double)probs[i].M * probs[i].N * 64.0;
        by += 4.0 * ((double)probs[i].M * 64.0 + (double)probs[i].N * 64.0 + 4.0 * (double)probs[i].M * probs[i].N);
    }
    TimedLaunch t(2, s, fl, by);
    return launch_gemm32_k64_gate_impl(probs, gates, nprob, s);
}

int launch_colsum(const float* const* X, float* const* out, const int64_t* M, const int32_t* N, const int32_t* ld,
                  int nprob, hipStream_t s) {
    IISAN_CHECK_SHAPE(nprob >= 1 && nprob <= 4, "colsum: 1..4 problems per launch");
    ColsumBatch b{};
    int64_t maxM = 0;
    int maxN = 0;
    for (int i = 0; i < nprob; ++i) {
        b.X[i] = X[i]; b.out[i] = out[i]; b.M[i] = M[i]; b.N[i] = N[i]; b.ld[i] = ld[i];
        if (M[i] > maxM) maxM = M[i];
        if (N[i] > maxN) maxN = N[i];
    }
    const int rows_per_block = 256;
    dim3 grid((unsigned)ceil_div(maxN, 64), (unsigned)ceil_div(maxM, rows_per_block), (unsigned)nprob);
    hipLaunchKernelGGL(colsum_kernel, grid, dim3(256), 0, s, b, rows_per_block);
    IISAN_LAUNCH_OK();
    return IISAN_OK;
}

extern "C" int iisan_gemm32(const float* A, const float* B, const float* bias, float* C, int64_t M, int32_t N, int64_t K,
                            int32_t ta, int32_t tb, int32_t relu, int32_t accumulate, void* stream) {
    Gemm32Prob p{};
    p.A = A; p.B = B; p.bias = bias; p.resid = nullptr; p.act_src = nullptr; p.C = C;
    p.M = M; p.N = N; p.K = K;
    p.lda = ta ? (int32_t)M : (int32_t)K;
    p.ldb = tb ? N : (int32_t)K;
    p.ldc = N; p.ldr = N;
    int flags = (ta ? G32_TA : 0) | (tb ? G32_TB : 0) | (relu ? G32_RELU : 0) | (accumulate ? G32_ACCUM : 0);
    return launch_gemm32(&p, 1, flags, (hipStream_t)stream);
}

extern "C" int iisan_linear_fwd(const float* x, const float* w, const float* b, float* y, int64_t M, int32_t K, int32_t N,
                                void* stream) {
    Gemm32Prob p{};
    p.A = x; p.B = w; p.bias = b; p.C = y; p.M = M; p.N = N; p.K = K; p.lda = K; p.ldb = K; p.ldc = N; p.ldr = N;
    return launch_gemm32(&p, 1, 0, (hipStream_t)stream);
}

extern "C" int iisan_linear_bwd(const float* x, const float* w, const float* dy, float* dx, float* dw, float* db,
                                int64_t M, int32_t K, int32_t N, void* stream) {
    hipStream_t s = (hipStream_t)stream;
    if (dx) {
        Gemm32Prob p{};
        p.A = dy; p.B = w; p.C = dx; p.M = M; p.N = K; p.K = N; p.lda = N; p.ldb = K; p.ldc = K; p.ldr = K;
        IISAN_TRY(launch_gemm32(&p, 1, G32_TB, s));
    }
    if (dw) {
        Gemm32Prob p{};
        p.A = dy; p.B = x; p.C = dw; p.M = N; p.N = K; p.K = M; p.lda = N; p.ldb = K; p.ldc = K; p.ldr = K;
        IISAN_TRY(launch_gemm32(&p, 1, G32_TA | G32_TB | G32_ACCUM, s));
    }
    if (db) {
        const float* X[1] = {dy};
        float* O[1] = {db};
        int64_t Ms[1] = {M};
        int32_t Ns[1] = {N}, lds[1] = {N};
        IISAN_TRY(launch_colsum(X, O, Ms, Ns, lds, 1, s));
    }
    return IISAN_OK;
}
```

### iisan_amd/csrc/sanb.hip

```cpp
#include "common.h"

namespace {


constexpr int R = 16;
constexpr int RD = 64;
constexpr int UST = RD + 4;
constexpr int NT = 256;

__device__ __forceinline__ float gate_of(const float* theta) { return 1.0f / (1.0f + __expf(-theta[0] / 0.1f)); }
__device__ __forceinline__ f4 mfma16(float a, float b, f4 c) { return __builtin_amdgcn_mfma_f32_16x16x4f32(a, b, c, 0, 0, 0); }

struct SanbTower {
    const float* a; const float* b; const float* prev;
    int64_t lda, ldb, ldp;
    const float* gate;
    int32_t D, type;
    const float* Wd; const float* bd;
    const float* Wu; const float* bu;
    float* F; float* U; float* A; float* O;
    const float* dO; const float* Upre;
    float* dU; float* dprev;
    float* da; float* db;
    float* dgate; float* dbu; float* dbd;
};
struct SanbArgs {
    SanbTower t[3];
    int64_t M;
    int32_t gelu;
};

__host__ __device__ constexpr int lds_floats(int D) { return R * (D + 4) + R * UST; }

template <int D>
__device__ __forceinline__ f4 narrow_product(const float* Xs, const float* __restrict__ W, int wave, int lane) {
    constexpr int FS = D + 4, NS = D / 16, PD = 8;
    const f4* xp = (const f4*)(Xs + (lane & 15) * FS + 4 * (lane >> 4));
    const f4* wp = (const f4*)(W + (int64_t)(wave * 16 + (lane & 15)) * D + 4 * (lane >> 4));
    f4 acc0 = {0.f, 0.f, 0.f, 0.f}, acc1 = {0.f, 0.f, 0.f, 0.f};
    f4 b[PD];
#pragma unroll
    for (int p = 0; p < PD; ++p) b[p] = wp[4 * p];
    static_assert(NS % PD == 0, "K steps");
    __builtin_amdgcn_sched_barrier(0);
    for (int s0 = 0; s0 < NS; s0 += PD) {
#pragma unroll
        for (int p = 0; p < PD; ++p) {
            const f4 a = xp[4 * (s0 + p)];
            const f4 bb = b[p];
            if (s0 + p + PD < NS) b[p] = wp[4 * (s0 + p + PD)];
            __builtin_amdgcn_sched_barrier(0);
            acc0 = mfma16(a[0], bb[0], acc0);
            acc1 = mfma16(a[1], bb[1], acc1);
            acc0 = mfma16(a[2], bb[2], acc0);
            acc1 = mfma16(a[3], bb[3], acc1);
            __builtin_amdgcn_sched_barrier(0);
        }
    }
    return acc0 + acc1;
}

template <int D>
__device__ __forceinline__ void wide_product(float* Ts, const float* Xs, const float* __restrict__ W, const float* __restrict__ bias,
                                             int wave, int lane) {
    constexpr int FS = D + 4;
    const int col = lane & 15, rg = lane >> 4;
    f4 a[4];
#pragma unroll
    for (int s = 0; s < 4; ++s) a[s] = *(const f4*)(Xs + col * UST + 16 * s + 4 * rg);
    const f4* wp = (const f4*)(W + (int64_t)(wave * (D / 4) + col) * RD + 4 * rg);
    f4 b0[4], b1[4];
#pragma unroll
    for (int s = 0; s < 4; ++s) { b0[s] = wp[4 * s]; b1[s] = wp[16 * 16 + 4 * s]; }
#pragma unroll 1
    for (int n0 = wave * (D / 4); n0 < (wave + 1) * (D / 4); n0 += 32) {
        f4 nb0[4], nb1[4];
        const bool more = n0 + 32 < (wave + 1) * (D / 4);
        if (more) {
#pragma unroll
            for (int s = 0; s < 4; ++s) { nb0[s] = wp[32 * 16 + 4 * s]; nb1[s] = wp[48 * 16 + 4 * s]; }
        }
        __builtin_amdgcn_sched_barrier(0);
        f4 c0, c1;
        float* t0 = Ts + (4 * rg) * FS + n0 + col;
        const float bi0 = bias ? bias[n0 + col] : 0.f, bi1 = bias ? bias[n0 + 16 + col] : 0.f;
#pragma unroll
        for (int r = 0; r < 4; ++r) { c0[r] = t0[r * FS] + bi0; c1[r] = t0[r * FS + 16] + bi1; }
#pragma unroll
        for (int s = 0; s < 4; ++s)
#pragma unroll
            for (int e = 0; e < 4; ++e) { c0 = mfma16(a[s][e], b0[s][e], c0); c1 = mfma16(a[s][e], b1[s][e], c1); }
#pragma unroll
        for (int r = 0; r < 4; ++r) { t0[r * FS] = c0[r]; t0[r * FS + 16] = c1[r]; }
        if (more) {
#pragma unroll
            for (int s = 0; s < 4; ++s) { b0[s] = nb0[s]; b1[s] = nb1[s]; }
        }
        wp += 32 * 16;
    }
}

template <int D>
__global__ __launch_bounds__(NT, 3) void sanb_fwd_kernel(SanbArgs args) {
    extern __shared__ __attribute__((aligned(16))) float smem[];
    const SanbTower& t = args.t[blockIdx.y];
    constexpr int FS = D + 4, d4 = D / 4;
    float* Fs = smem;
    float* As = smem + R * FS;
    const int tid = threadIdx.x, lane = tid & 63, wave = tid >> 6;
    const bool gated = t.gate != nullptr;
    const float g = gated ? gate_of(t.gate) : 1.0f;
    const int64_t ntiles = (args.M + R - 1) / R;
    for (int64_t tile = blockIdx.x; tile < ntiles; tile += gridDim.x) {
    const int64_t m0 = tile * R;

    constexpr int IT = R * d4 / NT, CH = IT % 4 == 0 ? 4 : (IT % 3 == 0 ? 3 : 1);
    for (int i0 = 0; i0 < IT; i0 += CH) {
        f4 av[CH], pv[CH], bv[CH];
#pragma unroll
        for (int j = 0; j < CH; ++j) {
            const int idx = tid + (i0 + j) * NT, row = idx / d4, c = (idx - row * d4) * 4;
            const int64_t m = m0 + row;
            av[j] = pv[j] = bv[j] = (f4){0.f, 0.f, 0.f, 0.f};
            if (m < args.M) {
                av[j] = *(const f4*)(t.a + m * t.lda + c);
                if (t.prev) pv[j] = *(const f4*)(t.prev + m * t.ldp + c);
                if (t.type == 1) bv[j] = *(const f4*)(t.b + m * t.ldb + c);
            }
        }
#pragma unroll
        for (int j = 0; j < CH; ++j) {
            const int idx = tid + (i0 + j) * NT, row = idx / d4, c = (idx - row * d4) * 4;
            const int64_t m = m0 + row;
            f4 o;
#pragma unroll
            for (int e = 0; e < 4; ++e) {
                if (t.type == 0) o[e] = gated ? g * av[j][e] + (1.f - g) * pv[j][e] : av[j][e] + pv[j][e];
                else o[e] = gated ? pv[j][e] + g * av[j][e] + (1.f - g) * bv[j][e] : pv[j][e] + av[j][e] + bv[j][e];
            }
            if (m < args.M) *(f4*)(t.F + m * D + c) = o;
            f2* fp = (f2*)(Fs + row * FS + c);
            fp[0] = (f2){o[0], o[1]};
            fp[1] = (f2){o[2], o[3]};
        }
    }
    __syncthreads();

    {
        const f4 u4 = narrow_product<D>(Fs, t.Wd, wave, lane);
        const int col = wave * 16 + (lane & 15);
        const float bd = t.bd[col];
#pragma unroll
        for (int r = 0; r < 4; ++r) {
            const int row = 4 * (lane >> 4) + r;
            const int64_t m = m0 + row;
            const float u = u4[r] + bd;
            const float a = args.gelu ? gelu_erf(u) : fmaxf(u, 0.f);
            As[row * UST + col] = a;
            if (m < args.M) {
                t.U[m * RD + col] = u;
                t.A[m * RD + col] = a;
            }
        }
    }
    __syncthreads();

    wide_product<D>(Fs, As, t.Wu, t.bu, wave, lane);
    __syncthreads();

    for (int idx = tid; idx < R * d4; idx += NT) {
        const int row = idx / d4, c = (idx - row * d4) * 4;
        const int64_t m = m0 + row;
        if (m >= args.M) continue;
        const f2* fp = (const f2*)(Fs + row * FS + c);
        const f2 lo = fp[0], hi = fp[1];
        *(f4*)(t.O + m * D + c) = (f4){lo[0], lo[1], hi[0], hi[1]};
    }
    __syncthreads();
    }
}

template <int D>
__global__ __launch_bounds__(NT, 3) void sanb_bwd_kernel(SanbArgs args) {
    extern __shared__ __attribute__((aligned(16))) float smem[];
    __shared__ float red[4];
    const SanbTower& t = args.t[blockIdx.y];
    constexpr int FS = D + 4, d4 = D / 4;
    float* Gs = smem;
    float* Ds = smem + R * FS;
    const int tid = threadIdx.x, lane = tid & 63, wave = tid >> 6;
    const bool gated = t.gate != nullptr;
    const float g = gated ? gate_of(t.gate) : 1.0f;
    const int64_t ntiles = (args.M + R - 1) / R;
    float gate_part = 0.f;
    float dbu_acc[D / NT], dbd_acc = 0.f;
#pragma unroll
    for (int i = 0; i < D / NT; ++i) dbu_acc[i] = 0.f;
    for (int64_t tile = blockIdx.x; tile < ntiles; tile += gridDim.x) {
    const int64_t m0 = tile * R;

    constexpr int IT = R * d4 / NT, CH = IT % 4 == 0 ? 4 : (IT % 3 == 0 ? 3 : 1);
    {
        f4 v[IT];
#pragma unroll
        for (int j = 0; j < IT; ++j) {
            const int idx = tid + j * NT, row = idx / d4, c = (idx - row * d4) * 4;
            const int64_t m = m0 + row;
            v[j] = (f4){0.f, 0.f, 0.f, 0.f};
            if (m < args.M) v[j] = *(const f4*)(t.dO + m * D + c);
        }
#pragma unroll
        for (int j = 0; j < IT; ++j) {
            const int idx = tid + j * NT, row = idx / d4, c = (idx - row * d4) * 4;
            f2* gp = (f2*)(Gs + row * FS + c);
            gp[0] = (f2){v[j][0], v[j][1]};
            gp[1] = (f2){v[j][2], v[j][3]};
        }
    }
    __syncthreads();

    if (t.dbu) {
#pragma unroll
        for (int i = 0; i < D / NT; ++i) {
            float s = 0.f;
#pragma unroll
            for (int row = 0; row < R; ++row) s += Gs[row * FS + tid + i * NT];
            dbu_acc[i] += s;
        }
    }

    {
        const f4 da = narrow_product<D>(Gs, t.Wd, wave, lane);
        const int col = wave * 16 + (lane & 15);
#pragma unroll
        for (int r = 0; r < 4; ++r) {
            const int row = 4 * (lane >> 4) + r;
            const int64_t m = m0 + row;
            float du = 0.f;
            if (m < args.M) {
                const float u = t.Upre[m * RD + col];
                du = da[r] * (args.gelu ? gelu_erf_grad(u) : (u > 0.f ? 1.f : 0.f));
                t.dU[m * RD + col] = du;
            }
            Ds[row * UST + col] = du;
        }
    }
    __syncthreads();
    if (t.dbd && tid < RD) {
        float s = 0.f;
#pragma unroll
        for (int row = 0; row < R; ++row) s += Ds[row * UST + tid];
        dbd_acc += s;
    }

    wide_product<D>(Gs, Ds, t.Wu, nullptr, wave, lane);
    __syncthreads();

    float part = 0.f;
    const float ca = gated ? g : 1.f, cb = gated ? 1.f - g : 1.f;
    for (int i0 = 0; i0 < IT; i0 += CH) {
        f4 av[CH], ov[CH];
#pragma unroll
        for (int j = 0; j < CH; ++j) {
            const int idx = tid + (i0 + j) * NT, row = idx / d4, c = (idx - row * d4) * 4;
            const int64_t m = m0 + row;
            av[j] = ov[j] = (f4){0.f, 0.f, 0.f, 0.f};
            if (gated && m < args.M) {
                av[j] = *(const f4*)(t.a + m * t.lda + c);
                if (t.type == 1) ov[j] = *(const f4*)(t.b + m * t.ldb + c);
                else if (t.prev) ov[j] = *(const f4*)(t.prev + m * t.ldp + c);
            }
        }
#pragma unroll
        for (int j = 0; j < CH; ++j) {
            const int idx = tid + (i0 + j) * NT, row = idx / d4, c = (idx - row * d4) * 4;
            const int64_t m = m0 + row;
            if (m >= args.M) continue;
            const f2* gp = (const f2*)(Gs + row * FS + c);
            const f2 lo = gp[0], hi = gp[1];
            const f4 df = {lo[0], lo[1], hi[0], hi[1]};
#pragma unroll
            for (int e = 0; e < 4; ++e) part += df[e] * (av[j][e] - ov[j][e]);
            if (t.da) *(f4*)(t.da + m * D + c) = (f4){ca * df[0], ca * df[1], ca * df[2], ca * df[3]};
            if (t.db) *(f4*)(t.db + m * D + c) = (f4){cb * df[0], cb * df[1], cb * df[2], cb * df[3]};
            if (t.dprev) {
                const float sc = (t.type == 0 && gated) ? cb : 1.f;
                *(f4*)(t.dprev + m * D + c) = (f4){sc * df[0], sc * df[1], sc * df[2], sc * df[3]};
            }
        }
    }
    gate_part += part;
    __syncthreads();
    }
    if (t.dbu) {
#pragma unroll
        for (int i = 0; i < D / NT; ++i) unsafeAtomicAdd(t.dbu + tid + i * NT, dbu_acc[i]);
    }
    if (t.dbd && tid < RD) unsafeAtomicAdd(t.dbd + tid, dbd_acc);
    if (gated) {
        gate_part = wave_sum(gate_part);
        if (lane == 0) red[wave] = gate_part;
        __syncthreads();
        if (tid == 0) atomicAdd(t.dgate, (red[0] + red[1] + red[2] + red[3]) * g * (1.f - g) / 0.1f);
    }
}

struct TransArgs { const float* in[6]; float* out[6]; int32_t rows[6], cols[6]; };
__global__ __launch_bounds__(256) void sanb_transpose_kernel(TransArgs a) {
    __shared__ float T[32][33];
    const int z = blockIdx.z;
    const int rows = a.rows[z], cols = a.cols[z];
    const int r0 = blockIdx.y * 32, c0 = blockIdx.x * 32;
    if (r0 >= rows || c0 >= cols) return;
    const int tx = threadIdx.x & 31, ty = threadIdx.x >> 5;
    for (int j = ty; j < 32; j += 8)
        if (r0 + j < rows && c0 + tx < cols) T[j][tx] = a.in[z][(int64_t)(r0 + j) * cols + c0 + tx];
    __syncthreads();
    for (int j = ty; j < 32; j += 8)
        if (c0 + j < cols && r0 + tx < rows) a.out[z][(int64_t)(c0 + j) * rows + r0 + tx] = T[tx][j];
}

size_t lds_bytes(int D) { return (size_t)lds_floats(D) * sizeof(float); }

}

bool sanb_fused_ok(int D, int down) { return down == RD && (D == 1024 || D == 768 || D == 512 || D == 256); }

static void fill(SanbTower& t, const SanbTowerDesc& d) {
    t.a = d.f.a; t.b = d.f.b; t.prev = d.f.prev; t.lda = d.f.lda; t.ldb = d.f.ldb; t.ldp = d.f.ldp; t.gate = d.f.gate; t.D = d.f.D; t.type = d.f.type;
    t.Wd = d.Wd; t.bd = d.bd; t.Wu = d.Wu; t.bu = d.bu; t.F = d.F; t.U = d.U; t.A = d.A; t.O = d.O;
    t.dO = d.dO; t.Upre = d.Upre; t.dU = d.dU; t.dprev = d.dprev; t.da = d.da; t.db = d.db; t.dgate = d.dgate; t.dbu = d.dbu; t.dbd = d.dbd;
}

template <bool BWD>
static int launch_sanb(const SanbTowerDesc* towers, int n, int64_t M, int gelu, hipStream_t s) {
    IISAN_CHECK_SHAPE(n >= 1 && n <= 3 && M > 0, "sanb: 1..3 towers per launch");
    SanbArgs a{};
    a.M = M; a.gelu = gelu;
    const int D = towers[0].f.D;
    for (int i = 0; i < n; ++i) {
        IISAN_CHECK_SHAPE(towers[i].f.D == D && sanb_fused_ok(D, RD), "sanb: towers of one launch must share a supported width");
        fill(a.t[i], towers[i]);
    }
    const int cus = iisan_cu_count();
    const int64_t ntile = ceil_div(M, R);
    const unsigned gx = (unsigned)(ntile > cus ? cus : ntile);
    const dim3 grid(gx, (unsigned)n), block(NT);
    const size_t lds = lds_bytes(D);
#define SANB_LAUNCH(DD)                                                                                                \
    do {                                                                                                               \
        auto k = BWD ? sanb_bwd_kernel<DD> : sanb_fwd_kernel<DD>;                                                      \
        static OncePerDevice attr;                                                                                     \
        if (attr.first())                                                                                              \
            IISAN_HIP_OK(hipFuncSetAttribute((const void*)k, hipFuncAttributeMaxDynamicSharedMemorySize, (int)lds_bytes(DD))); \
        hipLaunchKernelGGL(k, grid, block, lds, s, a);                                                                 \
    } while (0)
    switch (D) {
        case 256: SANB_LAUNCH(256); break;
        case 512: SANB_LAUNCH(512); break;
        case 768: SANB_LAUNCH(768); break;
        case 1024: SANB_LAUNCH(1024); break;
        default: iisan_set_error("sanb: width %d", D); return IISAN_EBADSHAPE;
    }
#undef SANB_LAUNCH
    IISAN_LAUNCH_OK();
    return IISAN_OK;
}

static int64_t g_cnt_sanb_fwd = 0, g_cnt_sanb_bwd = 0;
IISAN_DEV_COUNTER(sanb_fused_fwd, g_cnt_sanb_fwd);
IISAN_DEV_COUNTER(sanb_fused_bwd, g_cnt_sanb_bwd);
int launch_sanb_fwd(const SanbTowerDesc* towers, int n, int64_t M, int gelu, hipStream_t s) { ++g_cnt_sanb_fwd; return launch_sanb<false>(towers, n, M, gelu, s); }
int launch_sanb_bwd(const SanbTowerDesc* towers, int n, int64_t M, int gelu, hipStream_t s) { ++g_cnt_sanb_bwd; return launch_sanb<true>(towers, n, M, gelu, s); }

int launch_sanb_transpose(const float* const* in, float* const* out, const int32_t* rows, const int32_t* cols, int n, hipStream_t s) {
    IISAN_CHECK_SHAPE(n >= 1 && n <= 6, "sanb_transpose: 1..6 matrices per launch");
    TransArgs a{};
    int mr = 0, mc = 0;
    for (int i = 0; i < n; ++i) {
        a.in[i] = in[i]; a.out[i] = out[i]; a.rows[i] = rows[i]; a.cols[i] = cols[i];
        if (rows[i] > mr) mr = rows[i];
        if (cols[i] > mc) mc = cols[i];
    }
    hipLaunchKernelGGL(sanb_transpose_kernel, dim3((unsigned)ceil_div(mc, 32), (unsigned)ceil_div(mr, 32), (unsigned)n), dim3(256), 0, s, a);
    IISAN_LAUNCH_OK();
    return IISAN_OK;
}
```

### iisan_amd/csrc/sidenet.hip

```cpp
#include "common.h"

namespace {

struct FuseTower {
    const float* a; const float* b; const float* prev;
    int64_t lda, ldb, ldp;
    const float* gate;
    float* F;
    float* da; float* db;
    float* dgate;
    int32_t D, type;
};
struct FuseArgs {
    FuseTower t[3];
    int64_t M;
};

__device__ __forceinline__ float gate_of(const float* theta) { return 1.0f / (1.0f + __expf(-theta[0] / 0.1f)); }

__global__ __launch_bounds__(256) void fuse_fwd_kernel(FuseArgs args) {
    const FuseTower& t = args.t[blockIdx.y];
    const int d4 = t.D / 4;
    const int64_t total = args.M * d4;
    const bool gated = t.gate != nullptr;
    const float g = gated ? gate_of(t.gate) : 1.0f;
    const int64_t i0 = (int64_t)blockIdx.x * blockDim.x + threadIdx.x, step = (int64_t)gridDim.x * blockDim.x;
    const int64_t dm = step / d4;
    const int dc = (int)(step - dm * d4);
    int64_t m = i0 / d4;
    int c4 = (int)(i0 - m * d4);
    for (int64_t i = i0; i < total; i += step, m += dm, c4 += dc) {
        if (c4 >= d4) { c4 -= d4; ++m; }
        const int c = c4 * 4;
        const f4 av = *(const f4*)(t.a + m * t.lda + c);
        f4 pv = {0.f, 0.f, 0.f, 0.f}, bv = {0.f, 0.f, 0.f, 0.f};
        if (t.prev) pv = *(const f4*)(t.prev + m * t.ldp + c);
        if (t.type == 1) bv = *(const f4*)(t.b + m * t.ldb + c);
        f4 o;
#pragma unroll
        for (int e = 0; e < 4; ++e) {
            if (t.type == 0) o[e] = gated ? g * av[e] + (1.f - g) * pv[e] : av[e] + pv[e];
            else o[e] = gated ? pv[e] + g * av[e] + (1.f - g) * bv[e] : pv[e] + av[e] + bv[e];
        }
        *(f4*)(t.F + m * t.D + c) = o;
    }
}

__global__ __launch_bounds__(256) void fuse_bwd_kernel(FuseArgs args) {
    __shared__ float red[4];
    const FuseTower& t = args.t[blockIdx.y];
    const int d4 = t.D / 4;
    const int64_t total = args.M * d4;
    const bool gated = t.gate != nullptr;
    const float g = gated ? gate_of(t.gate) : 1.0f;
    float part = 0.f;
    const int64_t i0 = (int64_t)blockIdx.x * blockDim.x + threadIdx.x, step = (int64_t)gridDim.x * blockDim.x;
    const int64_t dm = step / d4;
    const int dc = (int)(step - dm * d4);
    int64_t m = i0 / d4;
    int c4 = (int)(i0 - m * d4);
    constexpr int CH = 4;
    const float ca = gated ? g : 1.f, cb = gated ? 1.f - g : 1.f;
    for (int64_t i = i0; i < total; i += CH * step) {
        f4 df[CH], av[CH], ov[CH];
        int64_t mm[CH];
        int cc[CH];
#pragma unroll
        for (int j = 0; j < CH; ++j) {
            if (c4 >= d4) { c4 -= d4; ++m; }
            mm[j] = m; cc[j] = c4 * 4;
            df[j] = av[j] = ov[j] = (f4){0.f, 0.f, 0.f, 0.f};
            if (i + j * step < total) {
                df[j] = *(const f4*)(t.F + m * t.D + cc[j]);
                if (gated) {
                    av[j] = *(const f4*)(t.a + m * t.lda + cc[j]);
                    if (t.type == 1) ov[j] = *(const f4*)(t.b + m * t.ldb + cc[j]);
                    else if (t.prev) ov[j] = *(const f4*)(t.prev + m * t.ldp + cc[j]);
                }
            }
            m += dm; c4 += dc;
        }
#pragma unroll
        for (int j = 0; j < CH; ++j) {
            if (i + j * step >= total) continue;
#pragma unroll
            for (int e = 0; e < 4; ++e) part += df[j][e] * (av[j][e] - ov[j][e]);
            const int64_t o = mm[j] * t.D + cc[j];
            if (t.da) *(f4*)(t.da + o) = (f4){ca * df[j][0], ca * df[j][1], ca * df[j][2], ca * df[j][3]};
            if (t.db) *(f4*)(t.db + o) = (f4){cb * df[j][0], cb * df[j][1], cb * df[j][2], cb * df[j][3]};
            if (t.type == 0 && gated) *(f4*)(t.F + o) = (f4){cb * df[j][0], cb * df[j][1], cb * df[j][2], cb * df[j][3]};
        }
    }
    if (!gated) return;
    part = wave_sum(part);
    if ((threadIdx.x & 63) == 0) red[threadIdx.x >> 6] = part;
    __syncthreads();
    if (threadIdx.x == 0) atomicAdd(t.dgate, (red[0] + red[1] + red[2] + red[3]) * g * (1.f - g) / 0.1f);
}

struct Plan {
    int n[3];
    int D[3];
    int H[3];
    int r, E;
    int diff_cv, diff_t;
    bool align;
    bool text_wide;
    int p_adapter[3], p_gate[3], p_dp, p_fc[3], p_head[3], n_params;
    int wd(int z, int k) const { return p_adapter[z] + 4 * k; }
    int gate(int z, int k) const { return p_gate[z] + k; }
    int dpw(int i) const { return p_dp + 2 * i; }
};

int make_plan(const iisan_side_cfg* c, Plan& p) {
    IISAN_CHECK_SHAPE(c->n_side >= 1 && c->n_side <= IISAN_MAX_SIDE, "side_net: n_side %d out of range", c->n_side);
    const int n_t = c->versa ? c->n_side_text : c->n_side;
    IISAN_CHECK_SHAPE(n_t >= 1 && n_t <= IISAN_MAX_SIDE, "side_net: n_side_text %d out of range", n_t);
    IISAN_CHECK_SHAPE(c->dim_cv % 4 == 0 && c->dim_text % 4 == 0 && c->down % 4 == 0 && c->emb % 4 == 0,
                      "side_net: widths must be multiples of 4");
    IISAN_CHECK_SHAPE(c->versa || c->dim_cv == c->dim_text, "side_net: towers of different width (%d vs %d) need versa = 1 "
                      "(Code_Cached_Asym)", c->dim_cv, c->dim_text);
    p.n[0] = c->n_side; p.n[1] = n_t; p.n[2] = p.n[0] < p.n[1] ? p.n[0] : p.n[1];
    p.D[0] = c->dim_cv; p.D[1] = c->dim_text; p.D[2] = c->dim_cv < c->dim_text ? c->dim_cv : c->dim_text;
    p.r = c->down; p.E = c->emb;
    p.diff_cv = p.n[0] > p.n[1] ? p.n[0] - p.n[1] : 0;
    p.diff_t = p.n[1] > p.n[0] ? p.n[1] - p.n[0] : 0;
    p.align = c->versa && c->dim_cv != c->dim_text;
    p.text_wide = c->dim_text > c->dim_cv;
    if (c->versa) { p.H[0] = p.E; p.H[1] = p.E; p.H[2] = p.D[2]; }
    else { p.H[0] = p.D[0]; p.H[1] = p.D[1]; p.H[2] = p.D[2]; }
    int o = 0;
    for (int z = 0; z < 3; ++z) { p.p_adapter[z] = o; o += 4 * p.n[z]; }
    for (int z = 0; z < 3; ++z) { p.p_gate[z] = o; o += p.n[z]; }
    p.p_dp = o; if (p.align) o += 2 * p.n[2];
    for (int z = 0; z < 3; ++z) { p.p_fc[z] = o; o += 2; }
    for (int z = 0; z < 3; ++z) { p.p_head[z] = o; o += 2; }
    p.n_params = o;
    for (int k = 0; k < p.n[0]; ++k)
        IISAN_CHECK_SHAPE(c->tap_index[k] >= 0 && c->tap_index[k] < c->tap_stride_cv, "side_net: cv tap index %d outside the tap tensor", c->tap_index[k]);
    for (int k = 0; k < p.n[1]; ++k) {
        const int ti = c->versa ? c->tap_index_text[k] : c->tap_index[k];
        IISAN_CHECK_SHAPE(ti >= 0 && ti < c->tap_stride_text, "side_net: text tap index %d outside the tap tensor", ti);
    }
    return IISAN_OK;
}

struct SideBufs {
    float* F[IISAN_MAX_SIDE][3];
    float* U[IISAN_MAX_SIDE][3];
    float* A[IISAN_MAX_SIDE][3];
    float* O[IISAN_MAX_SIDE][3];
    float* DP[IISAN_MAX_SIDE];
    float* Y[3];
    float* dO[3];
    float* dY[3];
    float* dU[3];
    float* dDP[IISAN_MAX_SIDE];
    void* x3; size_t x3_bytes;
    float* WT[3][2];
    float* skws; size_t skws_floats;
    uint32_t* amax;
    uint32_t* x3z_f; uint32_t* zb; uint32_t* x3z_b;
    mutable uint32_t* x3z_next; mutable int x3z_left;
};
constexpr int X3Z_WORDS = 12, X3Z_SLOTS_F = IISAN_MAX_SIDE + 4, X3Z_SLOTS_B = IISAN_MAX_SIDE + 8, ZB_HEAD = 4;

int g_use_x3 = 1;
constexpr int64_t SANB_FUSED_MAX_ROWS = 4096;
int g_use_sanb = 1;
int g_dw_merge = 1;

uint64_t x3_route_word() {
    const float f = (float)gemm_x3_get_min_flops();
    uint32_t bits;
    memcpy(&bits, &f, 4);
    return ((uint64_t)(g_use_x3 ? 1 : 0) << 32) | bits;
}

size_t x3_need(const Plan& p, int64_t M) {
    if (!g_use_x3) return 0;
    size_t need = 0;
    int64_t gm[IISAN_MAX_SIDE], gn[IISAN_MAX_SIDE], gk[IISAN_MAX_SIDE];
    int ng = 0;
    auto consider = [&](int64_t m, int64_t n, int64_t k) {
        Gemm32Prob q{};
        q.M = m; q.N = (int32_t)n; q.K = k; q.lda = q.ldb = q.ldc = q.ldr = 4;
        if (gemm_x3_applicable(q, 0) && ng < IISAN_MAX_SIDE) { gm[ng] = m; gn[ng] = n; gk[ng] = k; ++ng; }
    };
    auto close_group = [&]() {
        for (int i = 0; i < ng; i += 8) {
            const size_t b = gemm_x3_group_ws_bytes(gm + i, gn + i, gk + i, ng - i < 8 ? ng - i : 8);
            if (b > need) need = b;
        }
        ng = 0;
    };
    for (int z = 0; z < 3; ++z) consider(M, p.H[z], p.D[z]);
    close_group();
    for (int z = 0; z < 3; ++z) consider(M, p.D[z], p.H[z]);
    close_group();
    for (int z = 0; z < 3; ++z) consider(p.H[z], p.D[z], M);
    close_group();
    if (p.align) {
        const int dw = p.text_wide ? p.D[1] : p.D[0];
        for (int i = 0; i < p.n[2]; ++i) consider(M, p.D[2], dw);
        close_group();
        for (int i = 0; i < p.n[2]; ++i) consider(p.D[2], dw, M);
        close_group();
    }
    return need;
}

void carve(WsCarver& c, SideBufs& b, const Plan& p, int64_t M) {
    for (int z = 0; z < 3; ++z)
        for (int k = 0; k < p.n[z]; ++k) {
            b.F[k][z] = c.take<float>((size_t)M * p.D[z]);
            b.U[k][z] = c.take<float>((size_t)M * p.r);
            b.A[k][z] = c.take<float>((size_t)M * p.r);
            b.O[k][z] = c.take<float>((size_t)M * p.D[z]);
        }
    for (int i = 0; i < p.n[2]; ++i) b.DP[i] = p.align ? c.take<float>((size_t)M * p.D[2]) : nullptr;
    for (int z = 0; z < 3; ++z) {
        b.Y[z] = c.take<float>((size_t)M * p.H[z]);
        b.dO[z] = c.take<float>((size_t)M * p.D[z]);
        b.dY[z] = c.take<float>((size_t)M * p.H[z]);
        b.dU[z] = c.take<float>((size_t)M * p.r);
    }
    for (int i = 0; i < p.n[2]; ++i) b.dDP[i] = p.align ? c.take<float>((size_t)M * p.D[2]) : nullptr;
    for (int z = 0; z < 3; ++z) {
        b.WT[z][0] = c.take<float>((size_t)p.D[z] * p.r);
        b.WT[z][1] = c.take<float>((size_t)p.D[z] * p.r);
    }
    b.skws_floats = (size_t)3 * 8 * align_up((size_t)M * p.r, 64);
    {
        size_t wg = 0;
        for (int z = 0; z < 3; ++z) wg += (size_t)2 * 32 * align_up((size_t)p.D[z] * p.r + p.D[z], 64);
        if (wg > b.skws_floats) b.skws_floats = wg;
    }
    b.skws = c.take<float>(b.skws_floats);
    {
        uint32_t* zf = c.take<uint32_t>(16 + IISAN_MAX_SIDE + X3Z_WORDS * X3Z_SLOTS_F);
        b.amax = zf; b.x3z_f = zf ? zf + 16 + IISAN_MAX_SIDE : nullptr;
        b.zb = c.take<uint32_t>(ZB_HEAD + X3Z_WORDS * X3Z_SLOTS_B);
        b.x3z_b = b.zb ? b.zb + ZB_HEAD : nullptr;
        b.x3z_next = nullptr; b.x3z_left = 0;
    }
    b.x3_bytes = x3_need(p, M);
    b.x3 = b.x3_bytes ? (void*)c.take<char>(b.x3_bytes) : nullptr;
}

int gemm_group(const Gemm32Prob* pr, int n, int flags, const SideBufs& b, hipStream_t s) {
    Gemm32Prob rest[IISAN_MAX_SIDE], big[IISAN_MAX_SIDE];
    int nr = 0, nb = 0;
    IISAN_CHECK_SHAPE(n <= IISAN_MAX_SIDE, "gemm_group: %d problems", n);
    for (int i = 0; i < n; ++i) {
        if (b.x3 && gemm_x3_applicable(pr[i], flags)) {
            Gemm32Prob q = pr[i];
            if (b.x3z_left > 0) { q.x3_zeroed = b.x3z_next; b.x3z_next += X3Z_WORDS; --b.x3z_left; }
            big[nb++] = q;
        }
        else rest[nr++] = pr[i];
    }
    if (nb > 1 || (nb == 1 && big[0].x3_zeroed)) {
        AmaxBatch ab{};
        int na = 0;
        auto want = [&](const float* x, bool trans, int64_t op_rows, int64_t K, int64_t ld, uint32_t* slot) {
            for (int k = 0; k < na; ++k) if (ab.out[k] == slot) return;
            if (na >= 16) return;
            ab.x[na] = x; ab.rows[na] = trans ? K : op_rows; ab.cols[na] = trans ? op_rows : K; ab.ld[na] = ld; ab.out[na] = slot;
            ++na;
        };
        for (int i = 0; i < nb; ++i) {
            Gemm32Prob& q = big[i];
            if (!q.x3_zeroed && !(q.amax_a && q.amax_b)) continue;
            uint32_t* pa = q.amax_a ? q.amax_a : q.x3_zeroed;
            uint32_t* pb = q.amax_b ? q.amax_b : q.x3_zeroed + 1;
            const bool full = na + 2 > 16;
            if (full) break;
            if (!q.amax_a_ready) want(q.A, (flags & G32_TA) != 0, q.M, q.K, q.lda, pa);
            if (!q.amax_b_ready) want(q.B, (flags & G32_TB) != 0, q.N, q.K, q.ldb, pb);
            q.amax_a = pa; q.amax_b = pb; q.amax_a_ready = 1; q.amax_b_ready = 1;
        }
        IISAN_TRY(launch_amax_batch(ab, na, s));
    }
    const int gmax = gemm_x3_group_max();
    for (int i = 0; i < nb; i += gmax) IISAN_TRY(launch_gemm_x3_group(big + i, nb - i < gmax ? nb - i : gmax, flags, b.x3, b.x3_bytes, s));
    if (nr > 1 && !(flags & G32_ACCUM)) {
        int64_t kmin = INT64_MAX;
        for (int i = 0; i < nr; ++i) kmin = rest[i].K < kmin ? rest[i].K : kmin;
        for (int i = 0; i < nr;) {
            if (rest[i].N <= 64 && rest[i].K >= 4096 && rest[i].K >= 4 * kmin) {
                IISAN_TRY(launch_gemm32(&rest[i], 1, flags & ~G32_HINT_B_EXACT16, s));
                for (int k = i; k + 1 < nr; ++k) rest[k] = rest[k + 1];
                --nr;
            } else ++i;
        }
    }
    for (int i = 0; i < nr; i += 4)
        IISAN_TRY(launch_gemm32(rest + i, nr - i < 4 ? nr - i : 4, flags & ~G32_HINT_B_EXACT16, s));
    return IISAN_OK;
}

Gemm32Prob prob(const float* A, int lda, const float* B, int ldb, const float* bias, float* C, int ldc, int64_t M, int N,
                int64_t K, const float* resid = nullptr, int ldr = 0, const float* act_src = nullptr) {
    Gemm32Prob p{};
    p.A = A; p.B = B; p.bias = bias; p.resid = resid; p.act_src = act_src; p.C = C;
    p.M = M; p.N = N; p.K = K; p.lda = lda; p.ldb = ldb; p.ldc = ldc; p.ldr = ldr ? ldr : ldc;
    return p;
}

unsigned ew_grid(int64_t M, int D) {
    const int64_t b = ceil_div(M * (D / 4), 256);
    return (unsigned)(b < 4096 ? b : 4096);
}

struct StepMap {
    int nact; int z[3]; int k[3]; int mm_i;
};
StepMap step_map(const Plan& p, int g) {
    StepMap s{};
    const int diff = p.diff_cv + p.diff_t;
    if (g < diff) {
        s.nact = 1; s.z[0] = p.diff_cv ? 0 : 1; s.k[0] = g; s.mm_i = -1;
    } else {
        const int i = g - diff;
        s.nact = 3; s.mm_i = i;
        s.z[0] = 0; s.k[0] = i + p.diff_cv;
        s.z[1] = 1; s.k[1] = i + p.diff_t;
        s.z[2] = 2; s.k[2] = i;
    }
    return s;
}

struct ScratchGuard {
    ScratchGuard(float* p, size_t n) { gemm32_set_scratch(p, n); }
    ~ScratchGuard() { gemm32_set_scratch(nullptr, 0); }
};

void fill(FuseTower& t, const FuseOperands& f) {
    t.a = f.a; t.b = f.b; t.prev = f.prev; t.lda = f.lda; t.ldb = f.ldb; t.ldp = f.ldp; t.gate = f.gate; t.D = f.D; t.type = f.type;
}
K64Gate k64_gate(const FuseOperands& f) {
    K64Gate g{};
    g.gate = f.gate; g.ga = f.a; g.ldga = f.lda;
    if (f.type == 1) { g.go = f.b; g.ldgo = f.ldb; }
    else { g.go = f.prev; g.ldgo = f.ldp; }
    g.scale_prev = f.type == 0 ? 1 : 0;
    return g;
}

bool step_fusable(const Plan& p, const StepMap& sm, int64_t M) {
    if (!g_use_sanb || (g_use_sanb == 1 && M >= SANB_FUSED_MAX_ROWS)) return false;
    const int D = p.D[sm.z[0]];
    for (int a = 0; a < sm.nact; ++a)
        if (p.D[sm.z[a]] != D) return false;
    return sanb_fused_ok(D, p.r);
}

struct Ctx {
    const iisan_side_cfg* cfg; Plan p; SideBufs b;
    const float* taps[2]; int64_t M;
    const void* const* params;
    void* const* grads;
    hipStream_t s;
    const float* W(int i) const { return (const float*)params[i]; }
    float* G(int i) const { return (float*)grads[i]; }
    int tap_idx(int z, int k) const { return (z == 1 && cfg->versa) ? cfg->tap_index_text[k] : cfg->tap_index[k]; }
    int64_t tap_ld(int z) const { return (int64_t)(z == 0 ? cfg->tap_stride_cv : cfg->tap_stride_text) * p.D[z]; }
    const float* tap(int z, int k) const { return taps[z] + (int64_t)tap_idx(z, k) * p.D[z]; }
    int first_idx(int z) const { return (z == 1 && cfg->versa) ? cfg->first_index_text : cfg->first_index; }
    FuseOperands fuse_operands(int z, int k, const StepMap& sm) const {
        FuseOperands t{};
        t.D = p.D[z];
        t.gate = cfg->gated ? W(p.gate(z, k)) : nullptr;
        t.prev = nullptr; t.ldp = p.D[z];
        if (k > 0) t.prev = b.O[k - 1][z];
        else if (cfg->remove_first && z != 2) { t.prev = taps[z] + (int64_t)first_idx(z) * p.D[z]; t.ldp = tap_ld(z); }
        if (z != 2) {
            t.type = 0; t.a = tap(z, k); t.lda = tap_ld(z); t.b = nullptr; t.ldb = 0;
        } else {
            t.type = 1;
            const int kc = sm.k[0], kt = sm.k[1];
            t.a = tap(0, kc); t.lda = tap_ld(0);
            t.b = tap(1, kt); t.ldb = tap_ld(1);
            if (p.align) {
                if (p.text_wide) { t.b = b.DP[k]; t.ldb = p.D[2]; }
                else { t.a = b.DP[k]; t.lda = p.D[2]; }
            }
        }
        return t;
    }
    Gemm32Prob fc_prob(int z) const { return prob(b.O[p.n[z] - 1][z], p.D[z], W(p.p_fc[z]), p.D[z], W(p.p_fc[z] + 1), b.Y[z], p.H[z], M, p.H[z], p.D[z]); }
    Gemm32Prob align_prob(int i) const {
        const int zw = p.text_wide ? 1 : 0, kw = step_map(p, p.diff_cv + p.diff_t + i).k[zw];
        return prob(tap(zw, kw), (int)tap_ld(zw), W(p.dpw(i)), p.D[zw], W(p.dpw(i) + 1), b.DP[i], p.D[2], M, p.D[2], p.D[zw]);
    }

    int fwd_dim_align(bool taps_preset) const {
        Gemm32Prob pd[IISAN_MAX_SIDE];
        for (int i = 0; i < p.n[2]; ++i) {
            pd[i] = align_prob(i);
            pd[i].amax_a = b.amax + 9 + i;
            pd[i].amax_a_ready = taps_preset ? 1 : 0;
            pd[i].exact16_a = taps_preset ? 1 : 0;
        }
        return gemm_group(pd, p.n[2], 0, b, s);
    }

    int fwd_step_fused(const StepMap& sm) const {
        SanbTowerDesc td[3];
        for (int a = 0; a < sm.nact; ++a) {
            const int z = sm.z[a], k = sm.k[a];
            td[a] = SanbTowerDesc{};
            td[a].f = fuse_operands(z, k, sm);
            td[a].Wd = W(p.wd(z, k)); td[a].bd = W(p.wd(z, k) + 1); td[a].Wu = W(p.wd(z, k) + 2); td[a].bu = W(p.wd(z, k) + 3);
            td[a].F = b.F[k][z]; td[a].U = b.U[k][z]; td[a].A = b.A[k][z]; td[a].O = b.O[k][z];
        }
        return launch_sanb_fwd(td, sm.nact, M, cfg->gelu, s);
    }

    int fwd_step_separate(const StepMap& sm) const {
        const int na = sm.nact;
        FuseOperands fo[3];
        for (int a = 0; a < na; ++a) fo[a] = fuse_operands(sm.z[a], sm.k[a], sm);
        Gemm32Prob pr[3];
        bool fed = false;
        if (p.r == 64) {
            N64FDesc nd[3];
            for (int a = 0; a < na; ++a) {
                const int z = sm.z[a], k = sm.k[a];
                nd[a] = N64FDesc{};
                nd[a].f = fo[a];
                nd[a].F = b.F[k][z]; nd[a].W = W(p.wd(z, k)); nd[a].ldw = p.D[z]; nd[a].bias = W(p.wd(z, k) + 1);
                nd[a].U = b.U[k][z]; nd[a].A = b.A[k][z]; nd[a].M = M; nd[a].K = p.D[z];
            }
            if (gemm32_n64f_ok(nd, na)) {
                IISAN_TRY(launch_gemm32_n64f(nd, na, cfg->gelu, s));
                fed = true;
            }
        }
        if (!fed) {
            FuseArgs fa{};
            fa.M = M;
            int maxD = 0;
            for (int a = 0; a < na; ++a) {
                const int z = sm.z[a], k = sm.k[a];
                fill(fa.t[a], fo[a]);
                fa.t[a].F = b.F[k][z];
                if (p.D[z] > maxD) maxD = p.D[z];
                pr[a] = prob(b.F[k][z], p.D[z], W(p.wd(z, k)), p.D[z], W(p.wd(z, k) + 1), b.A[k][z], p.r, M, p.r, p.D[z], nullptr, 0, b.U[k][z]);
            }
            hipLaunchKernelGGL(fuse_fwd_kernel, dim3(ew_grid(M, maxD), na), dim3(256), 0, s, fa);
            IISAN_LAUNCH_OK();
            IISAN_TRY(launch_gemm32(pr, na, (cfg->gelu ? G32_GELU : G32_RELU) | G32_PREACT, s));
        }
        for (int a = 0; a < na; ++a) {
            const int z = sm.z[a], k = sm.k[a];
            pr[a] = prob(b.A[k][z], p.r, W(p.wd(z, k) + 2), p.r, W(p.wd(z, k) + 3), b.O[k][z], p.D[z], M, p.D[z], p.r, b.F[k][z], p.D[z]);
        }
        return launch_gemm32(pr, na, 0, s);
    }

    int fwd_fc_head(float* item3) const {
        Gemm32Prob pr[3];
        for (int z = 0; z < 3; ++z) {
            pr[z] = fc_prob(z);
            pr[z].amax_a = b.amax + z;
            pr[z].amax_b = b.amax + 3 + z;
        }
        IISAN_TRY(gemm_group(pr, 3, 0, b, s));
        for (int z = 0; z < 3; ++z) pr[z] = prob(b.Y[z], p.H[z], W(p.p_head[z]), p.H[z], W(p.p_head[z] + 1), item3 + z * p.E, 3 * p.E, M, p.E, p.H[z]);
        return launch_gemm32(pr, 3, 0, s);
    }

    int bwd_fc_head(const float* d_item3) const {
        const int E = p.E;
        Gemm32Prob pr[3];
        const float* cs_x[3]; float* cs_o[3]; int64_t cs_m[3] = {M, M, M}; int32_t cs_n[3], cs_ld[3];
        for (int z = 0; z < 3; ++z) pr[z] = prob(d_item3 + z * E, 3 * E, W(p.p_head[z]), p.H[z], nullptr, b.dY[z], p.H[z], M, p.H[z], E);
        IISAN_TRY(launch_gemm32(pr, 3, G32_TB, s));
        for (int z = 0; z < 3; ++z) pr[z] = prob(d_item3 + z * E, 3 * E, b.Y[z], p.H[z], nullptr, G(p.p_head[z]), p.H[z], E, p.H[z], M);
        IISAN_TRY(launch_gemm32(pr, 3, G32_TA | G32_TB | G32_ACCUM, s));
        for (int z = 0; z < 3; ++z) { cs_x[z] = d_item3 + z * E; cs_o[z] = G(p.p_head[z] + 1); cs_n[z] = E; cs_ld[z] = 3 * E; }
        IISAN_TRY(launch_colsum(cs_x, cs_o, cs_m, cs_n, cs_ld, 3, s));
        IISAN_HIP_OK(hipMemsetAsync(b.zb, 0, (size_t)(ZB_HEAD + X3Z_WORDS * X3Z_SLOTS_B) * sizeof(uint32_t), s));
        b.x3z_next = b.x3z_b; b.x3z_left = X3Z_SLOTS_B;
        int fwd_x3[3];
        for (int z = 0; z < 3; ++z) fwd_x3[z] = (b.x3 && gemm_x3_applicable(fc_prob(z), 0)) ? 1 : 0;
        for (int z = 0; z < 3; ++z) {
            pr[z] = prob(b.dY[z], p.H[z], W(p.p_fc[z]), p.D[z], nullptr, b.dO[z], p.D[z], M, p.D[z], p.H[z]);
            pr[z].amax_a = b.zb + z;
            if (fwd_x3[z]) { pr[z].amax_b = b.amax + 3 + z; pr[z].amax_b_ready = 1; }
        }
        IISAN_TRY(gemm_group(pr, 3, G32_TB, b, s));
        int dy_ready[3];
        for (int z = 0; z < 3; ++z) dy_ready[z] = (b.x3 && gemm_x3_applicable(pr[z], G32_TB)) ? 1 : 0;
        for (int z = 0; z < 3; ++z) {
            pr[z] = prob(b.dY[z], p.H[z], b.O[p.n[z] - 1][z], p.D[z], nullptr, G(p.p_fc[z]), p.D[z], p.H[z], p.D[z], M);
            pr[z].amax_a = b.zb + z; pr[z].amax_a_ready = dy_ready[z];
            if (fwd_x3[z]) { pr[z].amax_b = b.amax + z; pr[z].amax_b_ready = 1; }
        }
        IISAN_TRY(gemm_group(pr, 3, G32_TA | G32_TB | G32_ACCUM, b, s));
        for (int z = 0; z < 3; ++z) { cs_x[z] = b.dY[z]; cs_o[z] = G(p.p_fc[z] + 1); cs_n[z] = p.H[z]; cs_ld[z] = p.H[z]; }
        return launch_colsum(cs_x, cs_o, cs_m, cs_n, cs_ld, 3, s);
    }

    int bwd_step_fused(const StepMap& sm) const {
        const int na = sm.nact, r = p.r;
        Gemm32Prob pr[3];
        for (int a = 0; a < na; ++a) {
            const int z = sm.z[a], k = sm.k[a];
            pr[a] = prob(b.dO[z], p.D[z], b.A[k][z], r, nullptr, G(p.wd(z, k) + 2), r, p.D[z], r, M);
        }
        IISAN_TRY(launch_gemm32(pr, na, G32_TA | G32_TB | G32_ACCUM, s));
        SanbTowerDesc td[3];
        const float* tin[6]; float* tout[6]; int32_t trows[6], tcols[6];
        for (int a = 0; a < na; ++a) {
            const int z = sm.z[a], k = sm.k[a];
            tin[2 * a] = W(p.wd(z, k)); tout[2 * a] = b.WT[z][0]; trows[2 * a] = p.r; tcols[2 * a] = p.D[z];
            tin[2 * a + 1] = W(p.wd(z, k) + 2); tout[2 * a + 1] = b.WT[z][1]; trows[2 * a + 1] = p.D[z]; tcols[2 * a + 1] = p.r;
            td[a] = SanbTowerDesc{};
            td[a].f = fuse_operands(z, k, sm);
            td[a].Wd = b.WT[z][1]; td[a].Wu = b.WT[z][0];
            td[a].dO = b.dO[z]; td[a].Upre = b.U[k][z]; td[a].dU = b.dU[z];
            td[a].dprev = k > 0 ? b.dO[z] : nullptr;
            td[a].dgate = cfg->gated ? G(p.gate(z, k)) : nullptr;
            td[a].dbu = G(p.wd(z, k) + 3); td[a].dbd = G(p.wd(z, k) + 1);
        }
        IISAN_TRY(launch_sanb_transpose(tin, tout, trows, tcols, 2 * na, s));
        IISAN_TRY(launch_sanb_bwd(td, na, M, cfg->gelu, s));
        for (int a = 0; a < na; ++a) {
            const int z = sm.z[a], k = sm.k[a];
            pr[a] = prob(b.dU[z], r, b.F[k][z], p.D[z], nullptr, G(p.wd(z, k)), p.D[z], r, p.D[z], M);
        }
        return launch_gemm32(pr, na, G32_TA | G32_TB | G32_ACCUM, s);
    }

    int bwd_step_separate(const StepMap& sm) const {
        const int na = sm.nact, r = p.r;
        Gemm32Prob pr[3];
        for (int a = 0; a < na; ++a) {
            const int z = sm.z[a], k = sm.k[a];
            pr[a] = prob(b.dO[z], p.D[z], W(p.wd(z, k) + 2), r, nullptr, b.dU[z], r, M, r, p.D[z], nullptr, 0, b.U[k][z]);
        }
        IISAN_TRY(launch_gemm32(pr, na, G32_TB | (cfg->gelu ? G32_MUL_GELU_GRAD : G32_MUL_RELU_MASK), s));
        {
            Gemm32Prob pw[6];
            for (int a = 0; a < na; ++a) {
                const int z = sm.z[a], k = sm.k[a];
                pw[a] = prob(b.dO[z], p.D[z], b.A[k][z], r, nullptr, G(p.wd(z, k) + 2), r, p.D[z], r, M);
                pw[a].colsum_a = G(p.wd(z, k) + 3);
                pw[na + a] = prob(b.dU[z], r, b.F[k][z], p.D[z], nullptr, G(p.wd(z, k)), p.D[z], r, p.D[z], M);
                pw[na + a].colsum_a = G(p.wd(z, k) + 1);
            }
            if (g_dw_merge) IISAN_TRY(launch_gemm32(pw, 2 * na, G32_TA | G32_TB | G32_ACCUM, s));
            else {
                IISAN_TRY(launch_gemm32(pw, na, G32_TA | G32_TB | G32_ACCUM, s));
                IISAN_TRY(launch_gemm32(pw + na, na, G32_TA | G32_TB | G32_ACCUM, s));
            }
        }
        const bool need_dp = sm.mm_i >= 0 && p.align;
        FuseOperands fo[3];
        for (int a = 0; a < na; ++a) {
            const int z = sm.z[a], k = sm.k[a];
            fo[a] = fuse_operands(z, k, sm);
            pr[a] = prob(b.dU[z], r, W(p.wd(z, k)), p.D[z], nullptr, b.dO[z], p.D[z], M, p.D[z], r, b.dO[z], p.D[z]);
        }
        if (cfg->gated) {
            K64Gate kg[3];
            for (int a = 0; a < na; ++a) {
                const int z = sm.z[a], k = sm.k[a];
                kg[a] = k64_gate(fo[a]);
                kg[a].dgate = G(p.gate(z, k));
                kg[a].store = k > 0 ? 1 : 0;
                if (z == 2 && need_dp) { kg[a].d2 = b.dDP[sm.mm_i]; kg[a].ldd2 = p.D[2]; kg[a].d2_is_b = p.text_wide ? 1 : 0; }
            }
            if (gemm32_k64_gate_ok(pr, kg, na))
                return launch_gemm32_k64_gate(pr, kg, na, s);
        }
        IISAN_TRY(launch_gemm32(pr, na, G32_TB, s));
        if (!cfg->gated && !need_dp) return IISAN_OK;
        FuseArgs fa{};
        fa.M = M;
        int maxD = 0;
        for (int a = 0; a < na; ++a) {
            const int z = sm.z[a], k = sm.k[a];
            fill(fa.t[a], fo[a]);
            fa.t[a].F = b.dO[z];
            fa.t[a].dgate = cfg->gated ? G(p.gate(z, k)) : nullptr;
            if (z == 2 && need_dp) { if (p.text_wide) fa.t[a].db = b.dDP[sm.mm_i]; else fa.t[a].da = b.dDP[sm.mm_i]; }
            if (p.D[z] > maxD) maxD = p.D[z];
        }
        unsigned gb = ew_grid(M, maxD);
        if (gb > 768) gb = 768;
        hipLaunchKernelGGL(fuse_bwd_kernel, dim3(gb, na), dim3(256), 0, s, fa);
        IISAN_LAUNCH_OK();
        return IISAN_OK;
    }

    int bwd_dim_align() const {
        Gemm32Prob pd[IISAN_MAX_SIDE];
        const float* X[IISAN_MAX_SIDE]; float* O[IISAN_MAX_SIDE]; int64_t Ms[IISAN_MAX_SIDE]; int32_t Ns[IISAN_MAX_SIDE], lds[IISAN_MAX_SIDE];
        const int zw = p.text_wide ? 1 : 0;
        for (int i = 0; i < p.n[2]; ++i) {
            const Gemm32Prob f = align_prob(i);
            pd[i] = prob(b.dDP[i], p.D[2], f.A, f.lda, nullptr, G(p.dpw(i)), p.D[zw], p.D[2], p.D[zw], M);
            if (b.x3 && gemm_x3_applicable(f, 0)) {
                pd[i].amax_b = b.amax + 9 + i; pd[i].amax_b_ready = 1;
                pd[i].exact16_b = cfg->taps_exact16 ? 1 : 0;
            }
            X[i] = b.dDP[i]; O[i] = G(p.dpw(i) + 1); Ms[i] = M; Ns[i] = p.D[2]; lds[i] = p.D[2];
        }
        IISAN_TRY(gemm_group(pd, p.n[2], G32_TA | G32_TB | G32_ACCUM | G32_HINT_B_EXACT16, b, s));
        for (int i = 0; i < p.n[2]; i += 4) IISAN_TRY(launch_colsum(X + i, O + i, Ms + i, Ns + i, lds + i, p.n[2] - i < 4 ? p.n[2] - i : 4, s));
        return IISAN_OK;
    }
};

int setup(Ctx& c, const iisan_side_cfg* cfg, const float* taps_cv, const float* taps_text, int64_t M,
          const void* const* params, void* ws, size_t ws_bytes, hipStream_t s, const char* who) {
    IISAN_CHECK_SHAPE(M > 0, "side_net: M must be positive");
    c.cfg = cfg;
    IISAN_TRY(make_plan(cfg, c.p));
    WsCarver w(ws, ws_bytes);
    carve(w, c.b, c.p, M);
    if (w.overflow || !ws) {
        iisan_set_error("%s: workspace too small (%zu < %zu)", who, ws_bytes, w.off);
        return IISAN_EWORKSPACE;
    }
    c.taps[0] = taps_cv; c.taps[1] = taps_text; c.M = M; c.params = params; c.grads = nullptr; c.s = s;
    return IISAN_OK;
}

}

IISAN_DEV_KNOB(sanb_fused, g_use_sanb);
IISAN_DEV_KNOB(sidenet_dw_merge, g_dw_merge);

static int g_x3_mode = 1;
IISAN_DEV_KNOB_FN(x3, g_x3_mode, (g_x3_mode = (int)v, g_use_x3 = v != 0, gemm_x3_set_min_flops(v == 2 ? 0.0 : -1.0)));

extern "C" size_t iisan_side_net_ws_bytes(const iisan_side_cfg* cfg, int64_t M) {
    Plan p;
    if (make_plan(cfg, p) != IISAN_OK) return 0;
    WsCarver c(nullptr, 0);
    SideBufs b;
    carve(c, b, p, M);
    return c.off;
}

extern "C" int32_t iisan_side_net_num_params(const iisan_side_cfg* cfg) {
    Plan p;
    if (make_plan(cfg, p) != IISAN_OK) return -1;
    return p.n_params;
}

extern "C" int iisan_side_net_fwd(const iisan_side_cfg* cfg, const float* taps_cv, const float* taps_text, int64_t M,
                                  const void* const* params, float* item3, void* ws, size_t ws_bytes, uint64_t* fwd_token,
                                  void* stream) {
    hipStream_t s = (hipStream_t)stream;
    Ctx c;
    IISAN_TRY(setup(c, cfg, taps_cv, taps_text, M, params, ws, ws_bytes, s, "side_net_fwd"));
    const Plan& p = c.p;
    SideBufs& b = c.b;
    ScratchGuard guard(b.skws, b.skws_floats);
    IISAN_CHECK_SHAPE(fwd_token != nullptr, "side_net_fwd: fwd_token must not be null");
    *fwd_token = 0x51DE000000000000ull ^ x3_route_word();
    IISAN_HIP_OK(hipMemsetAsync(b.amax, 0, (size_t)(16 + IISAN_MAX_SIDE + X3Z_WORDS * X3Z_SLOTS_F) * sizeof(uint32_t), s));
    b.x3z_next = b.x3z_f; b.x3z_left = X3Z_SLOTS_F;
    const bool taps_preset = cfg->taps_exact16 && p.align && p.n[2] > 0;
    if (taps_preset) IISAN_HIP_OK(hipMemsetD32Async((hipDeviceptr_t)(b.amax + 9), 0x46000000, (size_t)p.n[2], s));
    if (p.align && p.n[2] > 0) IISAN_TRY(c.fwd_dim_align(taps_preset));
    const int nsteps = p.diff_cv + p.diff_t + p.n[2];
    for (int g = 0; g < nsteps; ++g) {
        const StepMap sm = step_map(p, g);
        IISAN_TRY(step_fusable(p, sm, M) ? c.fwd_step_fused(sm) : c.fwd_step_separate(sm));
    }
    return c.fwd_fc_head(item3);
}

extern "C" int iisan_side_net_bwd(const iisan_side_cfg* cfg, const float* taps_cv, const float* taps_text, int64_t M,
                                  const void* const* params, const float* d_item3, void* const* grads, void* ws,
                                  size_t ws_bytes, uint64_t fwd_token, void* stream) {
    Ctx c;
    if ((fwd_token >> 48) != 0x51DE) {
        iisan_set_error("side_net_bwd: fwd_token %llx did not come from side_net_fwd", (unsigned long long)fwd_token);
        return IISAN_EBADSHAPE;
    }
    if ((fwd_token ^ 0x51DE000000000000ull) != x3_route_word()) {
        iisan_set_error("side_net_bwd: the split-operand routing (the x3 switch) changed since side_net_fwd filled this workspace");
        return IISAN_EBADSHAPE;
    }
    IISAN_TRY(setup(c, cfg, taps_cv, taps_text, M, params, ws, ws_bytes, (hipStream_t)stream, "side_net_bwd"));
    c.grads = grads;
    const Plan& p = c.p;
    ScratchGuard guard(c.b.skws, c.b.skws_floats);
    IISAN_TRY(c.bwd_fc_head(d_item3));
    for (int g = p.diff_cv + p.diff_t + p.n[2] - 1; g >= 0; --g) {
        const StepMap sm = step_map(p, g);
        const bool fused = step_fusable(p, sm, M) && !(sm.mm_i >= 0 && p.align);
        IISAN_TRY(fused ? c.bwd_step_fused(sm) : c.bwd_step_separate(sm));
    }
    if (p.align && p.n[2] > 0) IISAN_TRY(c.bwd_dim_align());
    return IISAN_OK;
}
```

Measured before the change: 23520 items/s.

## Defer side-network weight-gradient GEMMs into one grouped split-K launch after backward

In the side-network backward, the per-step weight-gradient GEMMs are no longer issued between the fused SANB backward steps. Each layer's dO/dU is kept in its own buffer, all weight transposes happen in one batched transpose, and every dW GEMM runs at the end in a single grouped split-K kernel followed by a grouped reduction. The aim is to cut many small launches and fill the GPU better, at the cost of extra workspace (capped at a budget) and extra partial-sum memory traffic. It also reworks the weight prefetch in wide_product and adds optional timeline stamps that compile only under a debug macro.

```diff
diff --git a/iisan_amd/csrc/common.h b/iisan_amd/csrc/common.h
--- a/iisan_amd/csrc/common.h
+++ b/iisan_amd/csrc/common.h
@@ -383,6 +383,8 @@
     G32_DROPOUT = 256,
 };
 int launch_gemm32(const Gemm32Prob* probs, int nprob, int flags, hipStream_t s);
+size_t gemm32_dw_groups_scratch_floats(const Gemm32Prob* probs, const int* gsize, int ngroups, size_t launch_scratch_floats);
+int launch_gemm32_dw_groups(const Gemm32Prob* probs, const int* gsize, int ngroups, float* scratch, size_t scratch_floats, hipStream_t s);
 int launch_colsum(const float* const* X, float* const* out, const int64_t* M, const int32_t* N, const int32_t* ld,
                   int nprob, hipStream_t s);
 
diff --git a/iisan_amd/csrc/gemm32.hip b/iisan_amd/csrc/gemm32.hip
--- a/iisan_amd/csrc/gemm32.hip
+++ b/iisan_amd/csrc/gemm32.hip
@@ -284,9 +284,8 @@
         }
 }
 
-__global__ __launch_bounds__(256, 2) void gemm32_dw_kernel(Gemm32Batch batch) {
-    __shared__ __attribute__((aligned(16))) float sm[2][2][64 * 64];
-    const Gemm32Prob& p = batch.p[blockIdx.z];
+template <class P>
+__device__ __forceinline__ void dw_tile(const P& p, float (&sm)[2][2][64 * 64], const int nsplit, const int y) {
     const int tiles_n = p.N >> 6;
     const int64_t tiles_m = p.M >> 6;
     if ((int64_t)blockIdx.x >= tiles_m * tiles_n) return;
@@ -295,8 +294,8 @@
     const int64_t m0 = tile_m * 64;
     const int n0 = tile_n * 64;
     const int64_t ktiles = p.K / TK;
-    const int64_t per = (ktiles + gridDim.y - 1) / gridDim.y;
-    const int64_t kt0 = (int64_t)blockIdx.y * per;
+    const int64_t per = (ktiles + nsplit - 1) / nsplit;
+    const int64_t kt0 = (int64_t)y * per;
     int64_t kt1 = kt0 + per;
     if (kt1 > ktiles) kt1 = ktiles;
     if (kt0 >= kt1) return;
@@ -374,7 +373,7 @@
         for (int r = 0; r < 4; ++r)
             *(f4*)(red + (16 * kq + 4 * r + e) * 64 + 4 * i16) = (f4){acc[e][0][r], acc[e][1][r], acc[e][2][r], acc[e][3][r]};
     __syncthreads();
-    float* const Cp = p.C + (int64_t)blockIdx.y * p.ksplit_stride;
+    float* const Cp = p.C + (int64_t)y * p.ksplit_stride;
     const float* all = &sm[0][0][0];
 #pragma unroll
     for (int q = 0; q < 4; ++q) {
@@ -395,6 +394,25 @@
             Cp[p.M * p.N + m0 + tid] = v;
         }
     }
+}
+
+__global__ __launch_bounds__(256, 2) void gemm32_dw_kernel(Gemm32Batch batch) {
+    __shared__ __attribute__((aligned(16))) float sm[2][2][64 * 64];
+    dw_tile(batch.p[blockIdx.z], sm, (int)gridDim.y, (int)blockIdx.y);
+}
+
+constexpr int DW_GROUP_MAX = 48;
+struct DwProb {
+    const float* A; const float* B; float* C; float* colsum_a;
+    int64_t M, K, ksplit_stride;
+    int32_t N, lda, ldb, ldc, splits, pad;
+};
+struct DwGroup { DwProb p[DW_GROUP_MAX]; };
+__global__ __launch_bounds__(256, 2) void gemm32_dw_grouped_kernel(DwGroup g) {
+    __shared__ __attribute__((aligned(16))) float sm[2][2][64 * 64];
+    const DwProb& p = g.p[blockIdx.z];
+    if ((int)blockIdx.y >= p.splits) return;
+    dw_tile(p, sm, p.splits, (int)blockIdx.y);
 }
 
 struct N64FProb {
@@ -729,6 +747,40 @@
     }
 }
 
+struct RedProb { const float* P; float* C; float* cs; int64_t stride, M; int32_t N, ldc, ns, pad; };
+struct ReduceGroup { RedProb p[DW_GROUP_MAX]; };
+__global__ __launch_bounds__(256) void gemm32_reduce_grouped_kernel(ReduceGroup rg) {
+    const RedProb& p = rg.p[blockIdx.z];
+    const int ks = p.ns;
+    const float* P = p.P;
+    const int64_t stride = p.stride, total = p.M * p.N;
+    if (p.cs) {
+        for (int64_t m = (int64_t)blockIdx.x * blockDim.x + threadIdx.x; m < p.M; m += (int64_t)gridDim.x * blockDim.x) {
+            float v = 0.f;
+            for (int y = 0; y < ks; ++y) v += P[(int64_t)y * stride + total + m];
+            p.cs[m] += v;
+        }
+    }
+    const int64_t total4 = total / 4;
+    const int n4 = p.N / 4;
+    for (int64_t i = (int64_t)blockIdx.x * blockDim.x + threadIdx.x; i < total4; i += (int64_t)gridDim.x * blockDim.x) {
+        const int64_t m = i / n4;
+        const int n = (int)(i - m * n4) * 4;
+        f4 acc[8];
+#pragma unroll
+        for (int u = 0; u < 8; ++u) acc[u] = (f4){0.f, 0.f, 0.f, 0.f};
+        int y = 0;
+        for (; y + 8 <= ks; y += 8) {
+#pragma unroll
+            for (int u = 0; u < 8; ++u) acc[u] += *(const f4*)(P + (int64_t)(y + u) * stride + 4 * i);
+        }
+        for (int u = 0; y < ks; ++y, ++u) acc[u] += *(const f4*)(P + (int64_t)y * stride + 4 * i);
+        f4 v = ((acc[0] + acc[1]) + (acc[2] + acc[3])) + ((acc[4] + acc[5]) + (acc[6] + acc[7]));
+        v += *(const f4*)(p.C + m * p.ldc + n);
+        *(f4*)(p.C + m * p.ldc + n) = v;
+    }
+}
+
 thread_local float* g_scratch = nullptr;
 thread_local size_t g_scratch_floats = 0;
 
@@ -1091,6 +1143,89 @@
     return launch_reduce(rb, nprob, pl.splitk, epi, s);
 }
 
+static int64_t g_cnt_dw_grouped = 0;
+IISAN_DEV_COUNTER(gemm32_dw_grouped, g_cnt_dw_grouped);
+static constexpr int DW_MAX_GROUPS = 2 * IISAN_MAX_SIDE;
+
+static bool plan_dw_groups(const Gemm32Prob* probs, const int* gsize, int ngroups, size_t launch_scratch_floats, int* splitk, int64_t* need) {
+    if (ngroups < 1 || ngroups > DW_MAX_GROUPS) return false;
+    *need = 0;
+    const Gemm32Prob* q = probs;
+    for (int g = 0; g < ngroups; q += gsize[g], ++g) {
+        if (gsize[g] < 1 || gsize[g] > G32_MAXP) return false;
+        const Gemm32Plan pl = plan_gemm32(q, gsize[g], G32_TA | G32_TB | G32_ACCUM, launch_scratch_floats);
+        if (pl.kernel != G32K_DW || pl.scratch != G32S_ADD_C) return false;
+        for (int i = 0; i < gsize[g]; ++i) {
+            if ((q[i].ldc & 3) != 0 || q[i].lda > (1 << 28) || q[i].ldb > (1 << 28)) return false;
+            *need += (int64_t)pl.splitk * partial_floats(q[i], true);
+        }
+        splitk[g] = pl.splitk;
+    }
+    return true;
+}
+
+size_t gemm32_dw_groups_scratch_floats(const Gemm32Prob* probs, const int* gsize, int ngroups, size_t launch_scratch_floats) {
+    int splitk[DW_MAX_GROUPS];
+    int64_t need = 0;
+    return plan_dw_groups(probs, gsize, ngroups, launch_scratch_floats, splitk, &need) ? (size_t)need : 0;
+}
+
+int launch_gemm32_dw_groups(const Gemm32Prob* probs, const int* gsize, int ngroups, float* scratch, size_t scratch_floats, hipStream_t s) {
+    int splitk[DW_MAX_GROUPS];
+    int64_t need = 0;
+    const bool grouped = scratch && plan_dw_groups(probs, gsize, ngroups, g_scratch ? g_scratch_floats : 0, splitk, &need) &&
+                         (size_t)need <= scratch_floats;
+    if (!grouped) {
+        const Gemm32Prob* q = probs;
+        for (int g = 0; g < ngroups; q += gsize[g], ++g) IISAN_TRY(launch_gemm32(q, gsize[g], G32_TA | G32_TB | G32_ACCUM, s));
+        return IISAN_OK;
+    }
+    int total = 0;
+    double fl = 0, by = 0;
+    for (int g = 0; g < ngroups; ++g) total += gsize[g];
+    for (int i = 0; i < total; ++i) {
+        fl += 2.0 * (double)probs[i].M * probs[i].N * (double)probs[i].K;
+        by += 4.0 * ((double)probs[i].M * probs[i].K + (double)probs[i].N * probs[i].K + (double)probs[i].M * probs[i].N);
+    }
+    TimedLaunch t(2, s, fl, by);
+    int sk[DW_MAX_GROUPS * G32_MAXP];
+    for (int g = 0, i = 0; g < ngroups; ++g)
+        for (int k = 0; k < gsize[g]; ++k) sk[i++] = splitk[g];
+    int64_t off = 0;
+    for (int i0 = 0; i0 < total; i0 += DW_GROUP_MAX) {
+        const int n = total - i0 < DW_GROUP_MAX ? total - i0 : DW_GROUP_MAX;
+        DwGroup dg{};
+        ReduceGroup rg{};
+        int64_t max_tiles = 0, max_mn = 0;
+        int max_split = 0;
+        for (int i = 0; i < n; ++i) {
+            const Gemm32Prob& q = probs[i0 + i];
+            DwProb& d = dg.p[i];
+            d.A = q.A; d.B = q.B; d.C = scratch + off; d.colsum_a = q.colsum_a;
+            d.M = q.M; d.K = q.K; d.ksplit_stride = partial_floats(q, true);
+            d.N = q.N; d.lda = q.lda; d.ldb = q.ldb; d.ldc = q.N; d.splits = sk[i0 + i];
+            RedProb& r = rg.p[i];
+            r.P = d.C; r.C = q.C; r.cs = q.colsum_a; r.stride = d.ksplit_stride; r.M = q.M; r.N = q.N; r.ldc = q.ldc;
+            r.ns = nonempty_splits(ceil_div(q.K, (int64_t)TK), d.splits);
+            if (r.ns > d.splits) r.ns = d.splits;
+            off += (int64_t)d.splits * d.ksplit_stride;
+            const int64_t tiles = (q.M >> 6) * (q.N >> 6);
+            if (tiles > max_tiles) max_tiles = tiles;
+            if (q.M * q.N > max_mn) max_mn = q.M * q.N;
+            if (d.splits > max_split) max_split = d.splits;
+        }
+        ++g_cnt_dw_grouped;
+        hipLaunchKernelGGL(gemm32_dw_grouped_kernel, dim3((unsigned)max_tiles, (unsigned)max_split, (unsigned)n), dim3(256), 0, s, dg);
+        IISAN_LAUNCH_OK();
+        int64_t blocks = ceil_div(max_mn, 256);
+        if (blocks > 2048) blocks = 2048;
+        hipLaunchKernelGGL(gemm32_reduce_grouped_kernel, dim3((unsigned)blocks, 1, (unsigned)n), dim3(256), 0, s, rg);
+        IISAN_LAUNCH_OK();
+    }
+    g_cnt_dw += ngroups;
+    return IISAN_OK;
+}
+
 extern "C" int32_t iisan_gemm32_plan(const int64_t* M, const int32_t* N, const int64_t* K, int32_t nprob, int32_t flags, int64_t scratch_floats,
                                      int32_t with_colsum, int32_t* plan12) {
     static float present[4];
diff --git a/iisan_amd/csrc/sanb.hip b/iisan_amd/csrc/sanb.hip
--- a/iisan_amd/csrc/sanb.hip
+++ b/iisan_amd/csrc/sanb.hip
@@ -24,6 +24,18 @@
     float* da; float* db;
     float* dgate; float* dbu; float* dbd;
 };
+#ifdef SANB_TIMELINE
+constexpr int SANB_STAMP_WGS = 1024;
+__device__ unsigned long long g_sanb_stamps[2][SANB_STAMP_WGS][8];
+#define SANB_STAMP(DIR, I, CLK)                                                                                        \
+    do {                                                                                                               \
+        const unsigned w_ = blockIdx.x + gridDim.x * blockIdx.y;                                                      \
+        if (threadIdx.x == 0 && w_ < (unsigned)SANB_STAMP_WGS && tile == (int64_t)blockIdx.x) g_sanb_stamps[DIR][w_][I] = CLK(); \
+    } while (0)
+#else
+#define SANB_STAMP(DIR, I, CLK) do {} while (0)
+#endif
+
 struct SanbArgs {
     SanbTower t[3];
     int64_t M;
@@ -63,38 +75,46 @@
 template <int D>
 __device__ __forceinline__ void wide_product(float* Ts, const float* Xs, const float* __restrict__ W, const float* __restrict__ bias,
                                              int wave, int lane) {
-    constexpr int FS = D + 4;
+    constexpr int FS = D + 4, NI = D / 4 / 32;
+    constexpr int WD = 1;
     const int col = lane & 15, rg = lane >> 4;
     f4 a[4];
 #pragma unroll
     for (int s = 0; s < 4; ++s) a[s] = *(const f4*)(Xs + col * UST + 16 * s + 4 * rg);
     const f4* wp = (const f4*)(W + (int64_t)(wave * (D / 4) + col) * RD + 4 * rg);
-    f4 b0[4], b1[4];
-#pragma unroll
-    for (int s = 0; s < 4; ++s) { b0[s] = wp[4 * s]; b1[s] = wp[16 * 16 + 4 * s]; }
+    const float* bp = bias ? bias + wave * (D / 4) + col : nullptr;
+    f4 wb[WD + 1][2][4];
+    float bi[WD + 1][2];
+#pragma unroll
+    for (int i = 0; i < WD; ++i) {
+        bi[i][0] = bp && i < NI ? bp[32 * i] : 0.f; bi[i][1] = bp && i < NI ? bp[32 * i + 16] : 0.f;
+#pragma unroll
+        for (int s = 0; s < 4; ++s)
+            if (i < NI) { wb[i][0][s] = wp[(32 * i) * 16 + 4 * s]; wb[i][1][s] = wp[(32 * i + 16) * 16 + 4 * s]; }
+    }
 #pragma unroll 1
-    for (int n0 = wave * (D / 4); n0 < (wave + 1) * (D / 4); n0 += 32) {
-        f4 nb0[4], nb1[4];
-        const bool more = n0 + 32 < (wave + 1) * (D / 4);
-        if (more) {
-#pragma unroll
-            for (int s = 0; s < 4; ++s) { nb0[s] = wp[32 * 16 + 4 * s]; nb1[s] = wp[48 * 16 + 4 * s]; }
+    for (int i = 0; i < NI; ++i) {
+        if (i + WD < NI) {
+            bi[WD][0] = bp ? bp[32 * (i + WD)] : 0.f; bi[WD][1] = bp ? bp[32 * (i + WD) + 16] : 0.f;
+#pragma unroll
+            for (int s = 0; s < 4; ++s) { wb[WD][0][s] = wp[(32 * WD) * 16 + 4 * s]; wb[WD][1][s] = wp[(32 * WD + 16) * 16 + 4 * s]; }
         }
         __builtin_amdgcn_sched_barrier(0);
         f4 c0, c1;
-        float* t0 = Ts + (4 * rg) * FS + n0 + col;
-        const float bi0 = bias ? bias[n0 + col] : 0.f, bi1 = bias ? bias[n0 + 16 + col] : 0.f;
-#pragma unroll
-        for (int r = 0; r < 4; ++r) { c0[r] = t0[r * FS] + bi0; c1[r] = t0[r * FS + 16] + bi1; }
+        float* t0 = Ts + (4 * rg) * FS + wave * (D / 4) + 32 * i + col;
+#pragma unroll
+        for (int r = 0; r < 4; ++r) { c0[r] = t0[r * FS] + bi[0][0]; c1[r] = t0[r * FS + 16] + bi[0][1]; }
 #pragma unroll
         for (int s = 0; s < 4; ++s)
 #pragma unroll
-            for (int e = 0; e < 4; ++e) { c0 = mfma16(a[s][e], b0[s][e], c0); c1 = mfma16(a[s][e], b1[s][e], c1); }
+            for (int e = 0; e < 4; ++e) { c0 = mfma16(a[s][e], wb[0][0][s][e], c0); c1 = mfma16(a[s][e], wb[0][1][s][e], c1); }
 #pragma unroll
         for (int r = 0; r < 4; ++r) { t0[r * FS] = c0[r]; t0[r * FS + 16] = c1[r]; }
-        if (more) {
-#pragma unroll
-            for (int s = 0; s < 4; ++s) { b0[s] = nb0[s]; b1[s] = nb1[s]; }
+#pragma unroll
+        for (int k = 0; k < WD; ++k) {
+            bi[k][0] = bi[k + 1][0]; bi[k][1] = bi[k + 1][1];
+#pragma unroll
+            for (int s = 0; s < 4; ++s) { wb[k][0][s] = wb[k + 1][0][s]; wb[k][1][s] = wb[k + 1][1][s]; }
         }
         wp += 32 * 16;
     }
@@ -113,6 +133,8 @@
     const int64_t ntiles = (args.M + R - 1) / R;
     for (int64_t tile = blockIdx.x; tile < ntiles; tile += gridDim.x) {
     const int64_t m0 = tile * R;
+    SANB_STAMP(0, 5, __builtin_amdgcn_s_memrealtime);
+    SANB_STAMP(0, 0, __builtin_amdgcn_s_memtime);
 
     constexpr int IT = R * d4 / NT, CH = IT % 4 == 0 ? 4 : (IT % 3 == 0 ? 3 : 1);
     for (int i0 = 0; i0 < IT; i0 += CH) {
@@ -145,6 +167,7 @@
         }
     }
     __syncthreads();
+    SANB_STAMP(0, 1, __builtin_amdgcn_s_memtime);
 
     {
         const f4 u4 = narrow_product<D>(Fs, t.Wd, wave, lane);
@@ -164,9 +187,11 @@
         }
     }
     __syncthreads();
+    SANB_STAMP(0, 2, __builtin_amdgcn_s_memtime);
 
     wide_product<D>(Fs, As, t.Wu, t.bu, wave, lane);
     __syncthreads();
+    SANB_STAMP(0, 3, __builtin_amdgcn_s_memtime);
 
     for (int idx = tid; idx < R * d4; idx += NT) {
         const int row = idx / d4, c = (idx - row * d4) * 4;
@@ -177,6 +202,8 @@
         *(f4*)(t.O + m * D + c) = (f4){lo[0], lo[1], hi[0], hi[1]};
     }
     __syncthreads();
+    SANB_STAMP(0, 4, __builtin_amdgcn_s_memtime);
+    SANB_STAMP(0, 6, __builtin_amdgcn_s_memrealtime);
     }
 }
 
@@ -198,6 +225,8 @@
     for (int i = 0; i < D / NT; ++i) dbu_acc[i] = 0.f;
     for (int64_t tile = blockIdx.x; tile < ntiles; tile += gridDim.x) {
     const int64_t m0 = tile * R;
+    SANB_STAMP(1, 5, __builtin_amdgcn_s_memrealtime);
+    SANB_STAMP(1, 0, __builtin_amdgcn_s_memtime);
 
     constexpr int IT = R * d4 / NT, CH = IT % 4 == 0 ? 4 : (IT % 3 == 0 ? 3 : 1);
     {
@@ -218,6 +247,7 @@
         }
     }
     __syncthreads();
+    SANB_STAMP(1, 1, __builtin_amdgcn_s_memtime);
 
     if (t.dbu) {
 #pragma unroll
@@ -246,6 +276,7 @@
         }
     }
     __syncthreads();
+    SANB_STAMP(1, 2, __builtin_amdgcn_s_memtime);
     if (t.dbd && tid < RD) {
         float s = 0.f;
 #pragma unroll
@@ -255,6 +286,7 @@
 
     wide_product<D>(Gs, Ds, t.Wu, nullptr, wave, lane);
     __syncthreads();
+    SANB_STAMP(1, 3, __builtin_amdgcn_s_memtime);
 
     float part = 0.f;
     const float ca = gated ? g : 1.f, cb = gated ? 1.f - g : 1.f;
@@ -291,6 +323,8 @@
     }
     gate_part += part;
     __syncthreads();
+    SANB_STAMP(1, 4, __builtin_amdgcn_s_memtime);
+    SANB_STAMP(1, 6, __builtin_amdgcn_s_memrealtime);
     }
     if (t.dbu) {
 #pragma unroll
@@ -305,7 +339,8 @@
     }
 }
 
-struct TransArgs { const float* in[6]; float* out[6]; int32_t rows[6], cols[6]; };
+constexpr int SANB_TRANS_MAX = 6 * IISAN_MAX_SIDE;
+struct TransArgs { const float* in[SANB_TRANS_MAX]; float* out[SANB_TRANS_MAX]; int32_t rows[SANB_TRANS_MAX], cols[SANB_TRANS_MAX]; };
 __global__ __launch_bounds__(256) void sanb_transpose_kernel(TransArgs a) {
     __shared__ float T[32][33];
     const int z = blockIdx.z;
@@ -324,6 +359,12 @@
 
 }
 
+#ifdef SANB_TIMELINE
+extern "C" int sanb_timeline_read(unsigned long long* dst) {
+    IISAN_HIP_OK(hipMemcpyFromSymbol(dst, HIP_SYMBOL(g_sanb_stamps), sizeof(unsigned long long) * 2 * SANB_STAMP_WGS * 8));
+    return IISAN_OK;
+}
+#endif
 bool sanb_fused_ok(int D, int down) { return down == RD && (D == 1024 || D == 768 || D == 512 || D == 256); }
 
 static void fill(SanbTower& t, const SanbTowerDesc& d) {
@@ -374,7 +415,7 @@
 int launch_sanb_bwd(const SanbTowerDesc* towers, int n, int64_t M, int gelu, hipStream_t s) { ++g_cnt_sanb_bwd; return launch_sanb<true>(towers, n, M, gelu, s); }
 
 int launch_sanb_transpose(const float* const* in, float* const* out, const int32_t* rows, const int32_t* cols, int n, hipStream_t s) {
-    IISAN_CHECK_SHAPE(n >= 1 && n <= 6, "sanb_transpose: 1..6 matrices per launch");
+    IISAN_CHECK_SHAPE(n >= 1 && n <= SANB_TRANS_MAX, "sanb_transpose: 1..%d matrices per launch", SANB_TRANS_MAX);
     TransArgs a{};
     int mr = 0, mc = 0;
     for (int i = 0; i < n; ++i) {
diff --git a/iisan_amd/csrc/sidenet.hip b/iisan_amd/csrc/sidenet.hip
--- a/iisan_amd/csrc/sidenet.hip
+++ b/iisan_amd/csrc/sidenet.hip
@@ -159,6 +159,10 @@
     void* x3; size_t x3_bytes;
     float* WT[3][2];
     float* skws; size_t skws_floats;
+    bool deferred;
+    float* dOL[IISAN_MAX_SIDE][3]; float* dUL[IISAN_MAX_SIDE][3];
+    float* WTL[IISAN_MAX_SIDE][3][2];
+    float* dwws; size_t dwws_floats;
     uint32_t* amax;
     uint32_t* x3z_f; uint32_t* zb; uint32_t* x3z_b;
     mutable uint32_t* x3z_next; mutable int x3z_left;
@@ -169,6 +173,8 @@
 constexpr int64_t SANB_FUSED_MAX_ROWS = 4096;
 int g_use_sanb = 1;
 int g_dw_merge = 1;
+int g_dw_deferred = 1;
+constexpr size_t SIDE_DEFERRED_BUDGET = (size_t)256 << 20;
 
 uint64_t x3_route_word() {
     const float f = (float)gemm_x3_get_min_flops();
@@ -210,6 +216,12 @@
     return need;
 }
 
+struct StepMap;
+StepMap step_map(const Plan& p, int g);
+bool step_fusable(const Plan& p, const StepMap& sm, int64_t M);
+bool all_steps_fused(const Plan& p, int64_t M);
+int dw_groups(const Plan& p, const SideBufs& b, int64_t M, void* const* grads, Gemm32Prob* pr, int* gsize);
+
 void carve(WsCarver& c, SideBufs& b, const Plan& p, int64_t M) {
     for (int z = 0; z < 3; ++z)
         for (int k = 0; k < p.n[z]; ++k) {
@@ -246,6 +258,32 @@
     }
     b.x3_bytes = x3_need(p, M);
     b.x3 = b.x3_bytes ? (void*)c.take<char>(b.x3_bytes) : nullptr;
+    b.deferred = false; b.dwws = nullptr; b.dwws_floats = 0;
+    memset(b.dOL, 0, sizeof b.dOL); memset(b.dUL, 0, sizeof b.dUL); memset(b.WTL, 0, sizeof b.WTL);
+    if (!g_dw_deferred || !all_steps_fused(p, M)) return;
+    for (int z = 0; z < 3; ++z) { b.dOL[p.n[z] - 1][z] = b.dO[z]; b.dUL[p.n[z] - 1][z] = b.dU[z]; }
+    Gemm32Prob pr[6 * IISAN_MAX_SIDE];
+    int gsize[2 * IISAN_MAX_SIDE];
+    const int ng = dw_groups(p, b, M, nullptr, pr, gsize);
+    const size_t dw_floats = gemm32_dw_groups_scratch_floats(pr, gsize, ng, b.skws_floats);
+    size_t extra = align_up(dw_floats * sizeof(float), 256);
+    for (int z = 0; z < 3; ++z)
+        extra += (size_t)(p.n[z] - 1) * (align_up((size_t)M * p.D[z] * 4, 256) + align_up((size_t)M * p.r * 4, 256)) +
+                 (size_t)p.n[z] * 2 * align_up((size_t)p.D[z] * p.r * 4, 256);
+    if (extra > SIDE_DEFERRED_BUDGET) return;
+    b.deferred = true;
+    for (int z = 0; z < 3; ++z) {
+        for (int k = 0; k + 1 < p.n[z]; ++k) {
+            b.dOL[k][z] = c.take<float>((size_t)M * p.D[z]);
+            b.dUL[k][z] = c.take<float>((size_t)M * p.r);
+        }
+        for (int k = 0; k < p.n[z]; ++k) {
+            b.WTL[k][z][0] = c.take<float>((size_t)p.D[z] * p.r);
+            b.WTL[k][z][1] = c.take<float>((size_t)p.D[z] * p.r);
+        }
+    }
+    b.dwws_floats = dw_floats;
+    b.dwws = dw_floats ? c.take<float>(dw_floats) : nullptr;
 }
 
 int gemm_group(const Gemm32Prob* pr, int n, int flags, const SideBufs& b, hipStream_t s) {
@@ -354,6 +392,33 @@
     for (int a = 0; a < sm.nact; ++a)
         if (p.D[sm.z[a]] != D) return false;
     return sanb_fused_ok(D, p.r);
+}
+
+bool all_steps_fused(const Plan& p, int64_t M) {
+    for (int g = 0; g < p.diff_cv + p.diff_t + p.n[2]; ++g) {
+        const StepMap sm = step_map(p, g);
+        if (!step_fusable(p, sm, M) || (sm.mm_i >= 0 && p.align)) return false;
+    }
+    return true;
+}
+
+int dw_groups(const Plan& p, const SideBufs& b, int64_t M, void* const* grads, Gemm32Prob* pr, int* gsize) {
+    int ng = 0, n = 0;
+    const int r = p.r;
+    for (int g = p.diff_cv + p.diff_t + p.n[2] - 1; g >= 0; --g) {
+        const StepMap sm = step_map(p, g);
+        for (int a = 0; a < sm.nact; ++a) {
+            const int z = sm.z[a], k = sm.k[a];
+            pr[n++] = prob(b.dOL[k][z], p.D[z], b.A[k][z], r, nullptr, grads ? (float*)grads[p.wd(z, k) + 2] : nullptr, r, p.D[z], r, M);
+        }
+        gsize[ng++] = sm.nact;
+        for (int a = 0; a < sm.nact; ++a) {
+            const int z = sm.z[a], k = sm.k[a];
+            pr[n++] = prob(b.dUL[k][z], r, b.F[k][z], p.D[z], nullptr, grads ? (float*)grads[p.wd(z, k)] : nullptr, p.D[z], r, p.D[z], M);
+        }
+        gsize[ng++] = sm.nact;
+    }
+    return ng;
 }
 
 struct Ctx {
@@ -535,6 +600,37 @@
         return launch_gemm32(pr, na, G32_TA | G32_TB | G32_ACCUM, s);
     }
 
+    int bwd_deferred() const {
+        const int nsteps = p.diff_cv + p.diff_t + p.n[2];
+        const float* tin[6 * IISAN_MAX_SIDE]; float* tout[6 * IISAN_MAX_SIDE]; int32_t trows[6 * IISAN_MAX_SIDE], tcols[6 * IISAN_MAX_SIDE];
+        int nt = 0;
+        for (int z = 0; z < 3; ++z)
+            for (int k = 0; k < p.n[z]; ++k) {
+                tin[nt] = W(p.wd(z, k)); tout[nt] = b.WTL[k][z][0]; trows[nt] = p.r; tcols[nt] = p.D[z]; ++nt;
+                tin[nt] = W(p.wd(z, k) + 2); tout[nt] = b.WTL[k][z][1]; trows[nt] = p.D[z]; tcols[nt] = p.r; ++nt;
+            }
+        IISAN_TRY(launch_sanb_transpose(tin, tout, trows, tcols, nt, s));
+        for (int g = nsteps - 1; g >= 0; --g) {
+            const StepMap sm = step_map(p, g);
+            SanbTowerDesc td[3];
+            for (int a = 0; a < sm.nact; ++a) {
+                const int z = sm.z[a], k = sm.k[a];
+                td[a] = SanbTowerDesc{};
+                td[a].f = fuse_operands(z, k, sm);
+                td[a].Wd = b.WTL[k][z][1]; td[a].Wu = b.WTL[k][z][0];
+                td[a].dO = b.dOL[k][z]; td[a].Upre = b.U[k][z]; td[a].dU = b.dUL[k][z];
+                td[a].dprev = k > 0 ? b.dOL[k - 1][z] : nullptr;
+                td[a].dgate = cfg->gated ? G(p.gate(z, k)) : nullptr;
+                td[a].dbu = G(p.wd(z, k) + 3); td[a].dbd = G(p.wd(z, k) + 1);
+            }
+            IISAN_TRY(launch_sanb_bwd(td, sm.nact, M, cfg->gelu, s));
+        }
+        Gemm32Prob pr[6 * IISAN_MAX_SIDE];
+        int gsize[2 * IISAN_MAX_SIDE];
+        const int ng = dw_groups(p, b, M, grads, pr, gsize);
+        return launch_gemm32_dw_groups(pr, gsize, ng, b.dwws, b.dwws_floats, s);
+    }
+
     int bwd_step_separate(const StepMap& sm) const {
         const int na = sm.nact, r = p.r;
         Gemm32Prob pr[3];
@@ -635,6 +731,7 @@
 
 IISAN_DEV_KNOB(sanb_fused, g_use_sanb);
 IISAN_DEV_KNOB(sidenet_dw_merge, g_dw_merge);
+IISAN_DEV_KNOB(sidenet_dw_deferred, g_dw_deferred);
 
 static int g_x3_mode = 1;
 IISAN_DEV_KNOB_FN(x3, g_x3_mode, (g_x3_mode = (int)v, g_use_x3 = v != 0, gemm_x3_set_min_flops(v == 2 ? 0.0 : -1.0)));
@@ -695,6 +792,7 @@
     const Plan& p = c.p;
     ScratchGuard guard(c.b.skws, c.b.skws_floats);
     IISAN_TRY(c.bwd_fc_head(d_item3));
+    if (c.b.deferred) return c.bwd_deferred();
     for (int g = p.diff_cv + p.diff_t + p.n[2] - 1; g >= 0; --g) {
         const StepMap sm = step_map(p, g);
         const bool fused = step_fusable(p, sm, M) && !(sm.mm_i >= 0 && p.align);
```

After: 23690 items/s, median of 4. About the same (+0.7%).
